# anguswilliams91/bpl-next

Measured on NVIDIA B200. Metric: logdensity_grad_match_evals_per_s, higher is better.
Workload: dtype f32

## Files before the change

bpl_next_b200/csrc/api.cu:

```cuda
#include <limits.h>
#include <stdarg.h>
#include <stdlib.h>
#include <string.h>

#include <algorithm>
#include <atomic>
#include <mutex>
#include <new>

#include "common.cuh"
#include "plan.h"
#include "problem.h"
#include "loo.h"
#include "score_grid.h"
#include "simulate.h"

namespace bplx {

static thread_local char g_err[1024] = "";
static std::atomic<unsigned long long> g_launches{0};

void set_error(const char* fmt, ...) {
  va_list ap;
  va_start(ap, fmt);
  vsnprintf(g_err, sizeof g_err, fmt, ap);
  va_end(ap);
}
void note_launch(int n) { g_launches.fetch_add((unsigned long long)n, std::memory_order_relaxed); }

static EnvSwitches g_env;
static std::once_flag g_env_once;
void reload_env_switches() {
  EnvSwitches e;
  e.no_pdl = getenv("BPLX_NO_PDL") != nullptr;
  e.nuts_generic = getenv("BPLX_NUTS_GENERIC") != nullptr;
  e.no_tail_split = getenv("BPLX_NO_TAIL_SPLIT") != nullptr;
  e.no_transpose = getenv("BPLX_NO_TRANSPOSE") != nullptr;
  if (const char* v = getenv("BPLX_TRANSPOSE_MIN_ELEMS")) e.transpose_min_elems = (size_t)atoll(v);
  if (const char* v = getenv("BPLX_SPLIT")) e.split = atoi(v);
  if (const char* v = getenv("BPLX_HOST_CHUNKS")) e.host_chunks = atoi(v);
  g_env = e;
}
const EnvSwitches& env_switches() {
  std::call_once(g_env_once, reload_env_switches);
  return g_env;
}

constexpr size_t kUploadSlack = (size_t)kMaxSplit * kMaxWarps * sizeof(EntryClip) + 64;
template <typename T>
static int upload(bplx_problem* p, const std::vector<T>& h, const T** out) {
  *out = nullptr;
  if (h.empty()) return BPLX_OK;
  void* d = nullptr;
  const size_t bytes = h.size() * sizeof(T);
  BPLX_CUDA(cudaMalloc(&d, bytes + kUploadSlack));
  p->dev_allocs.push_back(d);
  BPLX_CUDA(cudaMemcpy(d, h.data(), bytes, cudaMemcpyHostToDevice));
  BPLX_CUDA(cudaMemset(static_cast<unsigned char*>(d) + bytes, 0, kUploadSlack));
  *out = static_cast<const T*>(d);
  return BPLX_OK;
}

static float* mapped_or(float* host, float* fallback) {
  cudaPointerAttributes a{};
  if (cudaPointerGetAttributes(&a, host) != cudaSuccess) {
    cudaGetLastError();
    return fallback;
  }
  if (a.type == cudaMemoryTypeHost && a.devicePointer != nullptr) return static_cast<float*>(a.devicePointer);
  return fallback;
}

__global__ void __launch_bounds__(256) transpose_kernel(const float* __restrict__ in, float* __restrict__ out, int R, int Cc,
                                                        size_t ldi, size_t ldo) {
  __shared__ float tile[4][32][33];
  const int c0 = blockIdx.x * 32, r0 = blockIdx.y * 128;
  float v[4][4];
#pragma unroll
  for (int s = 0; s < 4; s++)
#pragma unroll
    for (int k = 0; k < 4; k++) {
      const int r = r0 + s * 32 + threadIdx.y + 8 * k, c = c0 + threadIdx.x;
      v[s][k] = (r < R && c < Cc) ? in[(size_t)r * ldi + c] : 0.0f;
    }
#pragma unroll
  for (int s = 0; s < 4; s++)
#pragma unroll
    for (int k = 0; k < 4; k++) tile[s][threadIdx.y + 8 * k][threadIdx.x] = v[s][k];
  __syncthreads();
#pragma unroll
  for (int s = 0; s < 4; s++)
#pragma unroll
    for (int k = 0; k < 4; k++) {
      const int c = c0 + threadIdx.y + 8 * k, r = r0 + s * 32 + threadIdx.x;
      if (r < R && c < Cc) out[(size_t)c * ldo + r] = tile[s][threadIdx.x][threadIdx.y + 8 * k];
    }
}
static int launch_transpose(const float* in, float* out, int R, int Cc, size_t ldi, size_t ldo, cudaStream_t s) {
  const dim3 grid((unsigned)((Cc + 31) / 32), (unsigned)((R + 127) / 128));
  BPLX_REQUIRE(grid.y <= 65535u, BPLX_E_UNSUPPORTED, "transpose of %d rows", R);
  transpose_kernel<<<grid, dim3(32, 8), 0, s>>>(in, out, R, Cc, ldi, ldo);
  BPLX_CUDA(cudaGetLastError());
  note_launch(1);
  return BPLX_OK;
}

static size_t align256(size_t n) { return (n + 255) / 256 * 256; }
static size_t transpose_room(const KernelParams& kp, int C) {
  if ((size_t)C * (size_t)kp.D < env_switches().transpose_min_elems) return 0;
  return 2 * (((size_t)C + 31) / 32 * 32) * (size_t)kp.D * sizeof(float);
}

static size_t workspace_bytes(const KernelParams& kp, int C) {
  const size_t Cpad = ((size_t)C + 31) / 32 * 32;
  if (kp.model == BPLX_DYNAMIC)
    return ((size_t)kp.G * kp.T * 2 + (kp.dyn_hyp_ws ? (size_t)kp.G * 16 : 0)) * Cpad * sizeof(float);
  if (kp.Cf <= 0) return 0;
  return (size_t)kp.V * Cpad * sizeof(float);
}

static int enqueue(const bplx_problem* p, int C, int layout, int ld, const float* theta, float* lp, float* grad,
                   float* corr_coef, void* ws, size_t ws_bytes, cudaStream_t stream, bool pdl = false, bool lik = false) {
  BPLX_REQUIRE(p != nullptr, BPLX_E_INVALID, "problem is NULL");
  BPLX_REQUIRE(C > 0, BPLX_E_INVALID, "num_chains must be positive (got %d)", C);
  BPLX_REQUIRE(theta && lp && grad, BPLX_E_INVALID, "theta, lp and grad must not be NULL");
  if (layout == BPLX_CHAIN_MAJOR && !env_switches().no_transpose) {
    const size_t base = align256(workspace_bytes(p->kp, C)), room = transpose_room(p->kp, C);
    if (room > 0 && ws != nullptr && ws_bytes >= base + room) {
      const int Dc = lik ? p->lik_D : p->kp.D;
      const size_t ldm = ld > 0 ? (size_t)ld : (size_t)Dc, Cpad = ((size_t)C + 31) / 32 * 32;
      BPLX_REQUIRE(ldm >= (size_t)Dc, BPLX_E_INVALID, "chain-major ld (%d) < D (%d)", ld, Dc);
      float* tin = reinterpret_cast<float*>(static_cast<char*>(ws) + base);
      float* tout = tin + Cpad * (size_t)p->kp.D;
      int rc = launch_transpose(theta, tin, C, Dc, ldm, Cpad, stream);
      if (rc != BPLX_OK) return rc;
      rc = enqueue(p, C, BPLX_CHAIN_MINOR, (int)Cpad, tin, lp, tout, corr_coef, ws, base, stream, pdl, lik);
      if (rc != BPLX_OK) return rc;
      return launch_transpose(tout, grad, Dc, C, Cpad, ldm, stream);
    }
  }
  KernelParams kp = p->kp;
  if (lik) {
    BPLX_REQUIRE(kp.model != BPLX_DYNAMIC, BPLX_E_UNSUPPORTED, "bplx_loglik_fwdbwd: DYNAMIC is not supported");
    kp.lik_only = 1;
    kp.off = p->lik_off;
    for (int i = 0; i < 12; i++) kp.hyper[i] = p->lik_hyper[i];
    kp.nhyper = p->lik_nhyper;
    kp.D = p->lik_D;
    kp.K = 0;
    kp.const_term = p->lik_const;
  }
  if (layout == BPLX_CHAIN_MAJOR) {
    kp.sd = 1;
    kp.sc = ld > 0 ? ld : kp.D;
    BPLX_REQUIRE(kp.sc >= kp.D, BPLX_E_INVALID, "chain-major ld (%d) < D (%d)", ld, kp.D);
  } else if (layout == BPLX_CHAIN_MINOR) {
    kp.sc = 1;
    kp.sd = ld > 0 ? ld : C;
    BPLX_REQUIRE(kp.sd >= C, BPLX_E_INVALID, "chain-minor ld (%d) < num_chains (%d)", ld, C);
  } else {
    BPLX_REQUIRE(false, BPLX_E_INVALID, "unknown layout %d", layout);
  }
  BPLX_REQUIRE((long long)kp.D * (long long)kp.sd + (long long)C * (long long)kp.sc < (1ll << 31), BPLX_E_UNSUPPORTED,
               "theta / grad of %d x %d elements exceed the 31-bit element index of the kernel", C, kp.D);
  const size_t need = workspace_bytes(kp, C);
  BPLX_REQUIRE(ws_bytes >= need && (need == 0 || ws != nullptr), BPLX_E_WORKSPACE,
               "workspace too small: %zu bytes given, %zu needed", ws_bytes, need);
  kp.C = C;
  kp.Cpad = (C + 31) / 32 * 32;
  kp.theta = theta;
  kp.lp = lp;
  kp.grad = grad;
  kp.corr_coef = corr_coef;
  kp.scratch = static_cast<float*>(ws);
  int si = 0;
  const int groups = (C + kChains - 1) / kChains;
  for (int i = kNumSplits - 1; i >= 1; i--)
    if (p->s1[i] && (1 << i) <= kp.split_hint && groups <= p->max_clusters[i]) {
      si = i;
      break;
    }
  if (const int want = env_switches().split) {
    for (int i = 0; i < kNumSplits; i++)
      if ((1 << i) == want && p->s1[i] && (i == 0 || p->max_clusters[i] > 0)) si = i;
  }
  auto use_split = [&](int i) {
    kp.split = 1 << i;
    kp.stream1 = p->s1[i];
    kp.stream2 = p->s2[i];
    kp.warp_b1 = p->wb1[i];
    kp.warp_b2 = p->wb2[i];
  };
  use_split(si);
  kp.group0 = 0;
  kp.ngroups = groups;
  if (kp.model == BPLX_DYNAMIC) return launch_logdensity_dynamic(kp, stream);
  int ti = 0;
  const int rest = p->sm_count > 0 ? groups % p->sm_count : 0;
  if (si == 0 && rest > 0 && rest < groups && !env_switches().split && !env_switches().no_tail_split) {
    for (int i = kNumSplits - 1; i >= 1; i--)
      if (p->s1[i] && (1 << i) <= kp.split_hint && rest <= p->max_clusters[i] && rest * (1 << i) <= p->sm_count) {
        ti = i;
        break;
      }
  }
  if (ti == 0) return launch_logdensity(kp, p->wb[si], stream, pdl);
  kp.ngroups = groups - rest;
  int rc = launch_logdensity(kp, p->wb[0], stream, pdl);
  if (rc != BPLX_OK) return rc;
  use_split(ti);
  kp.group0 = groups - rest;
  kp.ngroups = rest;
  return launch_logdensity(kp, p->wb[ti], stream, pdl);
}

}

using namespace bplx;

extern "C" {

int bplx_problem_create(const bplx_problem_desc* desc, bplx_problem** out) {
  BPLX_REQUIRE(desc && out, BPLX_E_INVALID, "desc / out is NULL");
  *out = nullptr;
  HostPlan hp;
  std::string err;
  int rc = build_plan(*desc, &hp, &err);
  if (rc != BPLX_OK) {
    set_error("%s", err.c_str());
    return rc;
  }
  bplx_problem* p = new (std::nothrow) bplx_problem();
  BPLX_REQUIRE(p, BPLX_E_NOMEM, "out of host memory");
  auto fail = [&](int code) {
    bplx_problem_destroy(p);
    return code;
  };
  if (cudaGetDevice(&p->device) != cudaSuccess) {
    set_error("cudaGetDevice failed: no usable CUDA device (bplx has no CPU fallback)");
    return fail(BPLX_E_CUDA);
  }
  p->kp = hp.kp;
  p->layout = hp.layout;
  p->lik_off = hp.lik_off;
  for (int i = 0; i < 12; i++) p->lik_hyper[i] = hp.lik_hyper[i];
  p->lik_nhyper = hp.lik_nhyper;
  p->lik_D = hp.lik_D;
  p->lik_const = hp.lik_const;
  p->lik_layout = hp.lik_layout;
  KernelParams& kp = p->kp;
#define UP(vec, ptr)                                 \
  if ((rc = upload(p, hp.vec, &(ptr))) != BPLX_OK) return fail(rc)
  UP(stream1, p->s1[0]);
  UP(stream2, p->s2[0]);
  UP(warp_b1, p->wb1[0]);
  UP(warp_b2, p->wb2[0]);
  for (int i = 1; i < kNumSplits; i++) {
    if (hp.more[i - 1].stream1.empty()) continue;
    UP(more[i - 1].stream1, p->s1[i]);
    UP(more[i - 1].stream2, p->s2[i]);
    UP(more[i - 1].warp_b1, p->wb1[i]);
    UP(more[i - 1].warp_b2, p->wb2[i]);
  }
  auto keep_bounds = [&](int i, const std::vector<uint32_t>& b1, const std::vector<uint32_t>& b2) {
    const size_t cap = sizeof(p->wb[i].b1) / sizeof(uint32_t);
    for (size_t k = 0; k < b1.size() && k < cap; k++) p->wb[i].b1[k] = b1[k];
    for (size_t k = 0; k < b2.size() && k < cap; k++) p->wb[i].b2[k] = b2[k];
  };
  keep_bounds(0, hp.warp_b1, hp.warp_b2);
  for (int i = 1; i < kNumSplits; i++) keep_bounds(i, hp.more[i - 1].warp_b1, hp.more[i - 1].warp_b2);
  kp.stream1 = p->s1[0];
  kp.stream2 = p->s2[0];
  kp.warp_b1 = p->wb1[0];
  kp.warp_b2 = p->wb2[0];
  kp.split = 1;
  UP(team_vptr, kp.team_vptr);
  UP(team_flags, kp.team_flags);
  UP(v_team, kp.v_team);
  UP(v_conf, kp.v_conf);
  UP(conf_vptr, kp.conf_vptr);
  UP(conf_vlist, kp.conf_vlist);
  UP(yexp, kp.yexp);
  UP(yteam, kp.yteam);
  UP(yconf, kp.yconf);
  UP(Xs, kp.Xs);
  UP(gw_tptr, kp.gw_tptr);
  UP(gw_tlist, kp.gw_tlist);
#undef UP
  rc = kp.model == BPLX_DYNAMIC ? logdensity_dynamic_set_attributes() : logdensity_set_attributes(kp);
  if (rc != BPLX_OK) return fail(rc);
  if (cudaDeviceGetAttribute(&p->sm_count, cudaDevAttrMultiProcessorCount, p->device) != cudaSuccess) p->sm_count = 0;
  p->max_clusters[0] = 1 << 30;
  if (kp.model != BPLX_DYNAMIC)
    for (int i = 1; i < kNumSplits; i++) p->max_clusters[i] = p->s1[i] ? logdensity_max_clusters(kp, 1 << i) : 0;
  p->stats[0] = desc->num_matches;
  p->stats[1] = hp.n1;
  p->stats[2] = hp.n1_padded;
  p->stats[3] = hp.n2;
  p->stats[4] = hp.n2_padded;
  p->stats[5] = kp.smem_total;
  p->stats[6] = kp.nwarps;
  p->stats[7] = kp.V;
  if (kp.model != BPLX_DYNAMIC) {
    p->warp_stats.assign((size_t)kp.nwarps * 12, 0);
    for (int phase = 0; phase < 2; phase++) {
      const std::vector<unsigned char>& S = phase ? hp.stream2 : hp.stream1;
      const std::vector<uint32_t>& wb = phase ? hp.warp_b2 : hp.warp_b1;
      const size_t esz = (phase == 0 && kp.clip) ? sizeof(EntryClip) : sizeof(Entry);
      const uint32_t minp = phase ? kp.min_piece2 : kp.min_piece1;
      for (int w = 0; w < kp.nwarps && w + 1 < (int)wb.size(); w++) {
        long long* o = &p->warp_stats[(size_t)w * 12 + phase * 6];
        const uint32_t len = wb[w + 1] - wb[w];
        o[5] = (len + kp.stage_bytes - 1) / kp.stage_bytes;
        for (uint32_t st = 0; st < len; st += kp.stage_bytes) {
          uint32_t a = wb[w] + st;
          const uint32_t aend = wb[w] + std::min(len, st + kp.stage_bytes);
          while (a + minp <= aend) {
            ListHdr H;
            memcpy(&H, &S[a], sizeof H);
            if (H.n0 + H.n1 + H.n2 == 0) break;
            const bool home = (H.kind & 1) == 0;
            if (phase == 0) {
              o[home ? 0 : 1]++;
              o[home ? 2 : 3] += H.n0;
            } else {
              o[0]++;
              o[1] += H.n0;
              o[2] += H.n1;
              o[3] += H.n2;
            }
            if (H.flags & kTeamFirst) o[4]++;
            a += (uint32_t)sizeof(ListHdr) + (uint32_t)((H.n0 + H.n1 + H.n2) * esz);
          }
        }
      }
    }
  }
  *out = p;
  return BPLX_OK;
}

void bplx_problem_destroy(bplx_problem* p) {
  if (!p) return;
  for (void* d : p->dev_allocs) cudaFree(d);
  if (p->d_theta) cudaFree(p->d_theta);
  if (p->d_out) cudaFree(p->d_out);
  if (p->d_ws) cudaFree(p->d_ws);
  if (p->d_tin) cudaFree(p->d_tin);
  if (p->d_tout) cudaFree(p->d_tout);
  if (p->host_stream) cudaStreamDestroy(p->host_stream);
  if (p->host_in) cudaStreamDestroy(p->host_in);
  if (p->host_out) cudaStreamDestroy(p->host_out);
  for (cudaEvent_t e : p->host_ev)
    if (e) cudaEventDestroy(e);
  delete p;
}

int bplx_num_params(const bplx_problem* p) { return p ? p->kp.D : BPLX_E_INVALID; }

const char* bplx_problem_layout(const bplx_problem* p) { return p ? p->layout.c_str() : ""; }

int bplx_problem_stats(const bplx_problem* p, long long* out, int n) {
  BPLX_REQUIRE(p && out, BPLX_E_INVALID, "problem / out is NULL");
  for (int i = 0; i < n && i < 8; i++) out[i] = p->stats[i];
  return n < 8 ? n : 8;
}

int bplx_problem_warp_stats(const bplx_problem* p, long long* out, int n) {
  BPLX_REQUIRE(p && out, BPLX_E_INVALID, "problem / out is NULL");
  const int have = (int)p->warp_stats.size();
  for (int i = 0; i < n && i < have; i++) out[i] = p->warp_stats[i];
  return n < have ? n : have;
}

size_t bplx_logdensity_workspace_bytes(const bplx_problem* p, int num_chains) {
  if (!p || num_chains <= 0) return 0;
  const size_t room = transpose_room(p->kp, num_chains);
  return room ? align256(workspace_bytes(p->kp, num_chains)) + room : workspace_bytes(p->kp, num_chains);
}

int bplx_logdensity_fwdbwd(const bplx_problem* p, int num_chains, int layout, int ld, const float* theta, float* lp,
                           float* grad, float* corr_coef, void* workspace, size_t workspace_bytes, void* stream) {
  return enqueue(p, num_chains, layout, ld, theta, lp, grad, corr_coef, workspace, workspace_bytes,
                 static_cast<cudaStream_t>(stream), true);
}

int bplx_loglik_num_inputs(const bplx_problem* p) {
  if (!p) return BPLX_E_INVALID;
  return p->kp.model == BPLX_DYNAMIC ? BPLX_E_UNSUPPORTED : p->lik_D;
}

const char* bplx_loglik_layout(const bplx_problem* p) { return p ? p->lik_layout.c_str() : ""; }

int bplx_loglik_fwdbwd(const bplx_problem* p, int num_chains, int layout, int ld, const float* tables, float* loglik,
                       float* grad, float* corr_coef, void* workspace, size_t workspace_bytes, void* stream) {
  return enqueue(p, num_chains, layout, ld, tables, loglik, grad, corr_coef, workspace, workspace_bytes,
                 static_cast<cudaStream_t>(stream), true, true);
}

int bplx_logdensity_fwdbwd_host(bplx_problem* p, int C, const float* theta, float* lp, float* grad, float* corr_coef) {
  BPLX_REQUIRE(p != nullptr, BPLX_E_INVALID, "problem is NULL");
  BPLX_REQUIRE(C > 0, BPLX_E_INVALID, "num_chains must be positive (got %d)", C);
  BPLX_REQUIRE(theta && lp && grad, BPLX_E_INVALID, "theta, lp and grad must not be NULL");
  std::lock_guard<std::mutex> lock(p->mu);
  BPLX_CUDA(cudaSetDevice(p->device));
  const size_t D = (size_t)p->kp.D;
  if (!p->host_stream) BPLX_CUDA(cudaStreamCreateWithFlags(&p->host_stream, cudaStreamNonBlocking));
  if (C > p->host_cap) {
    if (p->d_theta) cudaFree(p->d_theta);
    if (p->d_out) cudaFree(p->d_out);
    if (p->d_ws) cudaFree(p->d_ws);
    p->d_theta = p->d_out = nullptr;
    p->d_ws = nullptr;
    p->host_cap = 0;
    BPLX_CUDA(cudaMalloc(&p->d_theta, (size_t)C * D * sizeof(float)));
    BPLX_CUDA(cudaMalloc(&p->d_out, ((size_t)C * D + 2 * (size_t)C) * sizeof(float)));
    p->d_ws_bytes = workspace_bytes(p->kp, C);
    if (p->d_ws_bytes) BPLX_CUDA(cudaMalloc(&p->d_ws, p->d_ws_bytes));
    p->host_cap = C;
  }
  if (!p->host_in) {
    BPLX_CUDA(cudaStreamCreateWithFlags(&p->host_in, cudaStreamNonBlocking));
    BPLX_CUDA(cudaStreamCreateWithFlags(&p->host_out, cudaStreamNonBlocking));
    for (cudaEvent_t& e : p->host_ev) BPLX_CUDA(cudaEventCreateWithFlags(&e, cudaEventDisableTiming));
  }
  cudaStream_t s = p->host_stream;
  float* d_grad = p->d_out;
  float* d_lp = p->d_out + (size_t)C * D;
  float* d_cc = d_lp + C;
  const size_t payload = (size_t)C * D * sizeof(float);
  int nchunk = payload >= ((size_t)80 << 20) ? 8 : (payload >= ((size_t)16 << 20) ? 4 : (payload >= ((size_t)6 << 20) ? 2 : 1));
  while (nchunk > 1 && C / nchunk < 256) nchunk /= 2;
  if (const int want = env_switches().host_chunks)
    if (want == 1 || want == 2 || want == 4 || want == 8 || want == 16) nchunk = want;
  const bool native = (size_t)C * D >= std::max(env_switches().transpose_min_elems, (size_t)1 << 20) && !env_switches().no_transpose;
  if (nchunk == 1) {
    float* k_lp = mapped_or(lp, d_lp);
    float* k_cc = corr_coef ? mapped_or(corr_coef, d_cc) : d_cc;
    BPLX_CUDA(cudaMemcpyAsync(p->d_theta, theta, (size_t)C * D * sizeof(float), cudaMemcpyHostToDevice, s));
    int rc;
    if (native) {
      const int ldc = (C + 31) / 32 * 32;
      if (ldc > p->tr_cap) {
        if (p->d_tin) cudaFree(p->d_tin);
        if (p->d_tout) cudaFree(p->d_tout);
        p->d_tin = p->d_tout = nullptr;
        p->tr_cap = 0;
        BPLX_CUDA(cudaMalloc(&p->d_tin, (size_t)ldc * D * sizeof(float)));
        BPLX_CUDA(cudaMalloc(&p->d_tout, (size_t)ldc * D * sizeof(float)));
        p->tr_cap = ldc;
      }
      rc = launch_transpose(p->d_theta, p->d_tin, C, (int)D, D, (size_t)ldc, s);
      if (rc != BPLX_OK) return rc;
      rc = enqueue(p, C, BPLX_CHAIN_MINOR, ldc, p->d_tin, k_lp, p->d_tout, k_cc, p->d_ws, p->d_ws_bytes, s);
      if (rc != BPLX_OK) return rc;
      rc = launch_transpose(p->d_tout, d_grad, (int)D, C, (size_t)ldc, D, s);
    } else {
      rc = enqueue(p, C, BPLX_CHAIN_MAJOR, (int)D, p->d_theta, k_lp, d_grad, k_cc, p->d_ws, p->d_ws_bytes, s);
    }
    if (rc != BPLX_OK) return rc;
    BPLX_CUDA(cudaMemcpyAsync(grad, d_grad, (size_t)C * D * sizeof(float), cudaMemcpyDeviceToHost, s));
    if (k_lp == d_lp) BPLX_CUDA(cudaMemcpyAsync(lp, d_lp, (size_t)C * sizeof(float), cudaMemcpyDeviceToHost, s));
    if (corr_coef && k_cc == d_cc)
      BPLX_CUDA(cudaMemcpyAsync(corr_coef, d_cc, (size_t)C * sizeof(float), cudaMemcpyDeviceToHost, s));
    BPLX_CUDA(cudaStreamSynchronize(s));
    return BPLX_OK;
  }
  const int per = ((C + nchunk - 1) / nchunk + 31) / 32 * 32;
  if (native && per > p->tr_cap) {
    if (p->d_tin) cudaFree(p->d_tin);
    if (p->d_tout) cudaFree(p->d_tout);
    p->d_tin = p->d_tout = nullptr;
    p->tr_cap = 0;
    BPLX_CUDA(cudaMalloc(&p->d_tin, (size_t)per * D * sizeof(float)));
    BPLX_CUDA(cudaMalloc(&p->d_tout, (size_t)per * D * sizeof(float)));
    p->tr_cap = per;
  }
  int sizes[40], ns = 0, left = C;
  auto push = [&](int n) {
    n = n < left ? n : left;
    if (n > 0) sizes[ns++] = n, left -= n;
  };
  if (nchunk >= 4) {
    const int half = (per / 2 + 31) / 32 * 32;
    push(half);
    push(half);
    while (left > per) push(per);
    push((left / 2 + 31) / 32 * 32);
    push(left);
  } else {
    while (left > 0) push(per);
  }
  for (int k = 0, c0 = 0; k < ns; c0 += sizes[k], k++) {
    const int n = sizes[k];
    const size_t off = (size_t)c0 * D;
    BPLX_CUDA(cudaMemcpyAsync(p->d_theta + off, theta + off, (size_t)n * D * sizeof(float), cudaMemcpyHostToDevice, p->host_in));
    BPLX_CUDA(cudaEventRecord(p->host_ev[2 * k], p->host_in));
    BPLX_CUDA(cudaStreamWaitEvent(s, p->host_ev[2 * k], 0));
    int rc;
    if (native) {
      rc = launch_transpose(p->d_theta + off, p->d_tin, n, (int)D, D, (size_t)per, s);
      if (rc != BPLX_OK) return rc;
      rc = enqueue(p, n, BPLX_CHAIN_MINOR, per, p->d_tin, d_lp + c0, p->d_tout, d_cc + c0, p->d_ws, p->d_ws_bytes, s);
      if (rc != BPLX_OK) return rc;
      rc = launch_transpose(p->d_tout, d_grad + off, (int)D, n, (size_t)per, D, s);
    } else {
      rc = enqueue(p, n, BPLX_CHAIN_MAJOR, (int)D, p->d_theta + off, d_lp + c0, d_grad + off, d_cc + c0, p->d_ws,
                   p->d_ws_bytes, s);
    }
    if (rc != BPLX_OK) return rc;
    BPLX_CUDA(cudaEventRecord(p->host_ev[2 * k + 1], s));
    BPLX_CUDA(cudaStreamWaitEvent(p->host_out, p->host_ev[2 * k + 1], 0));
    BPLX_CUDA(cudaMemcpyAsync(grad + off, d_grad + off, (size_t)n * D * sizeof(float), cudaMemcpyDeviceToHost, p->host_out));
    BPLX_CUDA(cudaMemcpyAsync(lp + c0, d_lp + c0, (size_t)n * sizeof(float), cudaMemcpyDeviceToHost, p->host_out));
    if (corr_coef)
      BPLX_CUDA(cudaMemcpyAsync(corr_coef + c0, d_cc + c0, (size_t)n * sizeof(float), cudaMemcpyDeviceToHost, p->host_out));
  }
  BPLX_CUDA(cudaStreamSynchronize(p->host_out));
  return BPLX_OK;
}

static int check_sample_args(const bplx_samples* s, const bplx_fixtures* f, const char* what,
                             bool allow_no_fixtures = false) {
  BPLX_REQUIRE(s && f, BPLX_E_INVALID, "samples / fixtures is NULL");
  BPLX_REQUIRE(s->model >= BPLX_DIXON_COLES && s->model <= BPLX_NEUTRAL_WC, BPLX_E_UNSUPPORTED,
               "%s: model %d unsupported (DYNAMIC predict is unusable in the reference)", what, s->model);
  const bool fixtures = !(allow_no_fixtures && f->num_fixtures == 0);
  BPLX_REQUIRE(s->num_samples > 0 && s->num_teams > 0 && (f->num_fixtures > 0 || !fixtures), BPLX_E_INVALID,
               "%s: num_samples, num_teams and num_fixtures must be positive", what);
  BPLX_REQUIRE(s->attack && s->defence && s->corr_coef && (!fixtures || (f->home_team && f->away_team)), BPLX_E_INVALID,
               "%s: attack, defence, corr_coef, home_team, away_team must not be NULL", what);
  BPLX_REQUIRE(s->home_attack, BPLX_E_INVALID, "%s: home_attack (home advantage) must not be NULL", what);
  if (s->model == BPLX_NEUTRAL || s->model == BPLX_NEUTRAL_WC)
    BPLX_REQUIRE(s->away_attack && s->home_defence && s->away_defence, BPLX_E_INVALID,
                 "%s: neutral models need away_attack, home_defence, away_defence", what);
  if (s->model == BPLX_NEUTRAL_WC)
    BPLX_REQUIRE(s->confederation_strength && s->num_conferences > 0 && (!fixtures || (f->home_conf && f->away_conf)),
                 BPLX_E_INVALID, "%s: NEUTRAL_WC needs confederation_strength, home_conf, away_conf", what);
  return BPLX_OK;
}

static int check_grid_args(const bplx_samples* s, const bplx_fixtures* f, int max_goals) {
  const int rc = check_sample_args(s, f, "score grid");
  if (rc != BPLX_OK) return rc;
  BPLX_REQUIRE(max_goals >= 1 && max_goals <= 63, BPLX_E_INVALID, "max_goals must be in [1, 63] (got %d)", max_goals);
  return BPLX_OK;
}

static size_t grid_plan(const bplx_samples* s, const bplx_fixtures* f, int max_goals, GridParams* gp, const char** err) {
  gp->model = s->model;
  gp->S = s->num_samples;
  gp->T = s->num_teams;
  gp->Cf = s->model == BPLX_NEUTRAL_WC ? s->num_conferences : 0;
  gp->F = f->num_fixtures;
  gp->g = max_goals + 1;
  return score_grid_plan(gp, err);
}

size_t bplx_score_grid_workspace_bytes(const bplx_samples* s, const bplx_fixtures* f, int max_goals) {
  if (!s || !f || max_goals < 1 || s->num_samples <= 0 || s->num_teams <= 0 || f->num_fixtures <= 0) return 0;
  GridParams gp{};
  return grid_plan(s, f, max_goals, &gp, nullptr);
}

int bplx_score_grid(const bplx_samples* s, const bplx_fixtures* f, int max_goals, float scale, float* grid,
                    float* outcome, void* workspace, size_t workspace_bytes, void* stream) {
  return bplx_score_grid_ex(s, f, max_goals, scale, grid, outcome, workspace, workspace_bytes, stream, 0u);
}

int bplx_score_grid_ex(const bplx_samples* s, const bplx_fixtures* f, int max_goals, float scale, float* grid,
                       float* outcome, void* workspace, size_t workspace_bytes, void* stream, unsigned flags) {
  int rc = check_grid_args(s, f, max_goals);
  if (rc != BPLX_OK) return rc;
  BPLX_REQUIRE(grid != nullptr, BPLX_E_INVALID, "grid is NULL");
  GridParams gp{};
  const char* perr = nullptr;
  const size_t need = grid_plan(s, f, max_goals, &gp, &perr);
  BPLX_REQUIRE(need > 0, BPLX_E_UNSUPPORTED, "%s", perr ? perr : "score grid: unsupported shape");
  gp.scale = scale;
  BPLX_REQUIRE(workspace && workspace_bytes >= need, BPLX_E_WORKSPACE,
               "workspace too small: %zu bytes given, %zu needed", workspace_bytes, need);
  BPLX_REQUIRE((reinterpret_cast<uintptr_t>(workspace) & 15u) == 0, BPLX_E_INVALID, "workspace must be 16-byte aligned");
  gp.attack = s->attack;
  gp.defence = s->defence;
  gp.ha = s->home_attack;
  gp.aa = s->away_attack;
  gp.hd = s->home_defence;
  gp.ad = s->away_defence;
  gp.conf = s->confederation_strength;
  gp.corr = s->corr_coef;
  gp.home = f->home_team;
  gp.away = f->away_team;
  gp.hconf = f->home_conf;
  gp.aconf = f->away_conf;
  gp.nv = f->neutral_venue;
  gp.table = static_cast<float*>(workspace);
  gp.partial = reinterpret_cast<float*>(static_cast<unsigned char*>(workspace) +
                                        ((size_t)gp.S * gp.row_floats * 4 + 255) / 256 * 256);
  gp.grid = grid;
  gp.outcome = outcome;
  gp.reuse_tables = (flags & BPLX_GRID_REUSE_TABLES) ? 1 : 0;
  return launch_score_grid(gp, static_cast<cudaStream_t>(stream));
}

int bplx_score_grid_host(const bplx_samples* s, const bplx_fixtures* f, int max_goals, float scale, float* grid,
                         float* outcome) {
  int rc = check_grid_args(s, f, max_goals);
  if (rc != BPLX_OK) return rc;
  BPLX_REQUIRE(grid != nullptr, BPLX_E_INVALID, "grid is NULL");
  const size_t S = s->num_samples, T = s->num_teams, F = f->num_fixtures, g = max_goals + 1;
  const size_t Cf = s->model == BPLX_NEUTRAL_WC ? s->num_conferences : 0;
  for (size_t i = 0; i < F; i++) {
    BPLX_REQUIRE(f->home_team[i] < T && f->away_team[i] < T, BPLX_E_INVALID,
                 "score grid: team index out of range at fixture %zu (%u, %u; num_teams %zu)", i,
                 (unsigned)f->home_team[i], (unsigned)f->away_team[i], T);
    if (Cf)
      BPLX_REQUIRE(f->home_conf[i] < Cf && f->away_conf[i] < Cf, BPLX_E_INVALID,
                   "score grid: confederation index out of range at fixture %zu (%u, %u; num_conferences %zu)", i,
                   (unsigned)f->home_conf[i], (unsigned)f->away_conf[i], Cf);
  }
  std::vector<void*> allocs;
  auto cleanup = [&]() {
    for (void* d : allocs) cudaFree(d);
  };
  cudaStream_t st = nullptr;
  if (cudaStreamCreateWithFlags(&st, cudaStreamNonBlocking) != cudaSuccess) {
    set_error("cudaStreamCreate failed: no usable CUDA device (bplx has no CPU fallback)");
    return BPLX_E_CUDA;
  }
  rc = BPLX_OK;
  auto up = [&](const void* h, size_t bytes) -> void* {
    if (!h || rc != BPLX_OK) return nullptr;
    void* d = nullptr;
    if (cudaMalloc(&d, bytes) != cudaSuccess ||
        cudaMemcpyAsync(d, h, bytes, cudaMemcpyHostToDevice, st) != cudaSuccess) {
      set_error("score_grid_host: device allocation / copy of %zu bytes failed", bytes);
      rc = BPLX_E_CUDA;
      return nullptr;
    }
    allocs.push_back(d);
    return d;
  };
  bplx_samples ds = *s;
  bplx_fixtures df = *f;
  const size_t ha_w = s->model == BPLX_DIXON_COLES ? 1 : T;
  ds.attack = (const float*)up(s->attack, S * T * 4);
  ds.defence = (const float*)up(s->defence, S * T * 4);
  ds.home_attack = (const float*)up(s->home_attack, S * ha_w * 4);
  const bool neu = s->model == BPLX_NEUTRAL || s->model == BPLX_NEUTRAL_WC;
  ds.away_attack = neu ? (const float*)up(s->away_attack, S * T * 4) : nullptr;
  ds.home_defence = neu ? (const float*)up(s->home_defence, S * T * 4) : nullptr;
  ds.away_defence = neu ? (const float*)up(s->away_defence, S * T * 4) : nullptr;
  ds.confederation_strength = Cf ? (const float*)up(s->confederation_strength, S * Cf * 4) : nullptr;
  ds.corr_coef = (const float*)up(s->corr_coef, S * 4);
  df.home_team = (const uint16_t*)up(f->home_team, F * 2);
  df.away_team = (const uint16_t*)up(f->away_team, F * 2);
  df.home_conf = Cf ? (const uint8_t*)up(f->home_conf, F) : nullptr;
  df.away_conf = Cf ? (const uint8_t*)up(f->away_conf, F) : nullptr;
  df.neutral_venue = (neu && f->neutral_venue) ? (const uint8_t*)up(f->neutral_venue, F) : nullptr;
  const size_t ws_bytes = bplx_score_grid_workspace_bytes(s, f, max_goals);
  void *d_ws = nullptr, *d_grid = nullptr, *d_out = nullptr;
  if (rc == BPLX_OK) {
    if (cudaMalloc(&d_ws, ws_bytes) == cudaSuccess) allocs.push_back(d_ws); else rc = BPLX_E_NOMEM;
    if (cudaMalloc(&d_grid, F * g * g * 4) == cudaSuccess) allocs.push_back(d_grid); else rc = BPLX_E_NOMEM;
    if (outcome) {
      if (cudaMalloc(&d_out, F * 3 * 4) == cudaSuccess) allocs.push_back(d_out); else rc = BPLX_E_NOMEM;
    }
    if (rc != BPLX_OK) set_error("score_grid_host: out of device memory");
  }
  if (rc == BPLX_OK)
    rc = bplx_score_grid(&ds, &df, max_goals, scale, (float*)d_grid, (float*)d_out, d_ws, ws_bytes, st);
  if (rc == BPLX_OK) {
    cudaError_t e = cudaMemcpyAsync(grid, d_grid, F * g * g * 4, cudaMemcpyDeviceToHost, st);
    if (e == cudaSuccess && outcome) e = cudaMemcpyAsync(outcome, d_out, F * 3 * 4, cudaMemcpyDeviceToHost, st);
    if (e == cudaSuccess) e = cudaStreamSynchronize(st);
    if (e != cudaSuccess) {
      set_error("score_grid_host: %s", cudaGetErrorString(e));
      rc = BPLX_E_CUDA;
    }
  } else {
    cudaStreamSynchronize(st);
  }
  cleanup();
  cudaStreamDestroy(st);
  return rc;
}

static size_t pointwise_plan_for(const bplx_samples* s, const bplx_observations* o, PointwiseParams* pp, const char** err) {
  pp->gp.model = s->model;
  pp->gp.S = s->num_samples;
  pp->gp.T = s->num_teams;
  pp->gp.Cf = s->model == BPLX_NEUTRAL_WC ? s->num_conferences : 0;
  pp->gp.F = o->fixtures.num_fixtures;
  return pointwise_plan(pp, err);
}

size_t bplx_pointwise_loglik_workspace_bytes(const bplx_samples* s, const bplx_observations* obs) {
  if (!s || !obs || s->num_samples <= 0 || s->num_teams <= 0 || obs->fixtures.num_fixtures <= 0) return 0;
  PointwiseParams pp{};
  return pointwise_plan_for(s, obs, &pp, nullptr);
}

int bplx_pointwise_loglik(const bplx_samples* s, const bplx_observations* obs, float* loglik, size_t ld, double* stats,
                          void* workspace, size_t workspace_bytes, void* stream) {
  BPLX_REQUIRE(obs != nullptr, BPLX_E_INVALID, "observations is NULL");
  int rc = check_sample_args(s, &obs->fixtures, "pointwise log-likelihood");
  if (rc != BPLX_OK) return rc;
  BPLX_REQUIRE(obs->home_goals && obs->away_goals, BPLX_E_INVALID,
               "pointwise log-likelihood: home_goals and away_goals must not be NULL");
  BPLX_REQUIRE(stats != nullptr, BPLX_E_INVALID, "pointwise log-likelihood: stats is NULL");
  BPLX_REQUIRE(!loglik || ld >= (size_t)s->num_samples, BPLX_E_INVALID,
               "pointwise log-likelihood: ld (%zu) < num_samples (%d)", ld, s->num_samples);
  PointwiseParams pp{};
  const char* perr = nullptr;
  const size_t need = pointwise_plan_for(s, obs, &pp, &perr);
  BPLX_REQUIRE(need > 0, BPLX_E_UNSUPPORTED, "%s", perr ? perr : "pointwise log-likelihood: unsupported shape");
  BPLX_REQUIRE(workspace && workspace_bytes >= need, BPLX_E_WORKSPACE,
               "workspace too small: %zu bytes given, %zu needed", workspace_bytes, need);
  BPLX_REQUIRE((reinterpret_cast<uintptr_t>(workspace) & 15u) == 0, BPLX_E_INVALID, "workspace must be 16-byte aligned");
  GridParams& gp = pp.gp;
  gp.attack = s->attack;
  gp.defence = s->defence;
  gp.ha = s->home_attack;
  gp.aa = s->away_attack;
  gp.hd = s->home_defence;
  gp.ad = s->away_defence;
  gp.conf = s->confederation_strength;
  gp.corr = s->corr_coef;
  gp.home = obs->fixtures.home_team;
  gp.away = obs->fixtures.away_team;
  gp.hconf = obs->fixtures.home_conf;
  gp.aconf = obs->fixtures.away_conf;
  gp.nv = obs->fixtures.neutral_venue;
  gp.table = static_cast<float*>(workspace);
  pp.partial = reinterpret_cast<double*>(static_cast<unsigned char*>(workspace) +
                                         ((size_t)gp.S * gp.row_floats * 4 + 255) / 256 * 256);
  pp.hg = obs->home_goals;
  pp.ag = obs->away_goals;
  pp.ll = loglik;
  pp.ld = ld;
  pp.stats = stats;
  return launch_pointwise(pp, static_cast<cudaStream_t>(stream));
}

int bplx_psis_loo(const float* loglik, int num_matches, int num_samples, size_t ld, double r_eff, double* elpd_i,
                  double* pareto_k, void* workspace, size_t workspace_bytes, void* stream) {
  (void)workspace;
  (void)workspace_bytes;
  BPLX_REQUIRE(loglik && elpd_i && pareto_k, BPLX_E_INVALID, "psis loo: loglik, elpd_i and pareto_k must not be NULL");
  BPLX_REQUIRE(num_matches > 0 && num_samples > 0, BPLX_E_INVALID,
               "psis loo: num_matches and num_samples must be positive (got %d, %d)", num_matches, num_samples);
  BPLX_REQUIRE(ld >= (size_t)num_samples, BPLX_E_INVALID, "psis loo: ld (%zu) < num_samples (%d)", ld, num_samples);
  BPLX_REQUIRE(r_eff > 0.0 && r_eff <= 1e300, BPLX_E_INVALID, "psis loo: r_eff must be positive and finite (got %g)", r_eff);
  PsisParams pp{};
  pp.Mt = psis_tail_length(num_samples, r_eff);
  BPLX_REQUIRE(pp.Mt <= kPsisTailMax, BPLX_E_UNSUPPORTED,
               "psis loo: a tail of %d draws (ceil(min(0.2 S, 3 sqrt(S / r_eff)))) exceeds the kernel's limit of %d "
               "(BPLX_PSIS_MAX_TAIL)", pp.Mt, kPsisTailMax);
  pp.cap = 8;
  while (pp.cap < pp.Mt) pp.cap <<= 1;
  pp.ll = loglik;
  pp.ld = ld;
  pp.M = num_matches;
  pp.S = num_samples;
  pp.elpd = elpd_i;
  pp.khat = pareto_k;
  return launch_psis(pp, static_cast<cudaStream_t>(stream));
}

static size_t simulate_plan_for(const bplx_samples* s, const bplx_fixtures* f, SimParams* sp) {
  sp->gp.model = s->model;
  sp->gp.S = s->num_samples;
  sp->gp.T = s->num_teams;
  sp->gp.Cf = s->model == BPLX_NEUTRAL_WC ? s->num_conferences : 0;
  sp->gp.F = f->num_fixtures;
  return simulate_plan(sp);
}

size_t bplx_simulate_workspace_bytes(const bplx_samples* s, const bplx_fixtures* f, const bplx_table* t) {
  if (!s || !f || !t || s->num_samples <= 0 || s->num_teams <= 0 || f->num_fixtures <= 0) return 0;
  SimParams sp{};
  return simulate_plan_for(s, f, &sp);
}

static int simulate_setup(const bplx_samples* s, const bplx_fixtures* f, const uint8_t* home_slot,
                          const uint8_t* away_slot, const bplx_table* t, int max_goals, int sims_per_draw,
                          unsigned long long seed, long long first_draw, unsigned long long* position_counts,
                          unsigned long long* points_counts, uint8_t* positions, uint8_t* scores,
                          unsigned long long* invalid, const char* what, bool allow_no_fixtures, SimParams* out) {
  int rc = check_sample_args(s, f, what, allow_no_fixtures);
  if (rc != BPLX_OK) return rc;
  BPLX_REQUIRE(t != nullptr, BPLX_E_INVALID, "%s: table is NULL", what);
  BPLX_REQUIRE(t->num_slots <= BPLX_SIM_MAX_TEAMS, BPLX_E_UNSUPPORTED,
               "%s: %d table slots exceed the kernel's limit of %d (BPLX_SIM_MAX_TEAMS)", what, t->num_slots,
               BPLX_SIM_MAX_TEAMS);
  BPLX_REQUIRE(t->num_slots >= 1, BPLX_E_INVALID, "%s: the table needs at least one slot", what);
  BPLX_REQUIRE(t->num_positions >= 1 && t->num_positions <= t->num_slots && t->num_points_bins >= 1, BPLX_E_INVALID,
               "%s: num_positions must be in [1, num_slots] and num_points_bins >= 1 (got %d, %d)", what,
               t->num_positions, t->num_points_bins);
  BPLX_REQUIRE(t->points_win >= 1 && t->points_draw >= 0 && t->points_draw <= t->points_win, BPLX_E_INVALID,
               "%s: points must satisfy 0 <= points_draw <= points_win, points_win >= 1 (got %d, %d)", what,
               t->points_win, t->points_draw);
  BPLX_REQUIRE(t->start_points && t->start_goals_for && t->start_goals_against, BPLX_E_INVALID,
               "%s: start_points, start_goals_for and start_goals_against must not be NULL", what);
  BPLX_REQUIRE((home_slot && away_slot) || f->num_fixtures == 0, BPLX_E_INVALID,
               "%s: home_slot and away_slot must not be NULL", what);
  BPLX_REQUIRE(max_goals >= 1 && max_goals <= 63, BPLX_E_INVALID, "%s: max_goals must be in [1, 63] (got %d)", what,
               max_goals);
  BPLX_REQUIRE(sims_per_draw >= 1, BPLX_E_INVALID, "%s: sims_per_draw must be >= 1 (got %d)", what, sims_per_draw);
  BPLX_REQUIRE(first_draw >= 0 && first_draw + s->num_samples <= LLONG_MAX / sims_per_draw, BPLX_E_INVALID,
               "%s: first_draw must be >= 0 and (first_draw + num_samples) * sims_per_draw must fit 63 bits", what);
  BPLX_REQUIRE((long long)s->num_samples * sims_per_draw <= INT_MAX, BPLX_E_UNSUPPORTED,
               "%s: num_samples * sims_per_draw must be below 2^31 per call (got %lld): cut the draws into ranges",
               what, (long long)s->num_samples * sims_per_draw);
  BPLX_REQUIRE(position_counts && points_counts && invalid, BPLX_E_INVALID,
               "%s: position_counts, points_counts and invalid must not be NULL", what);
  SimParams& sp = *out;
  GridParams& gp = sp.gp;
  gp.attack = s->attack;
  gp.defence = s->defence;
  gp.ha = s->home_attack;
  gp.aa = s->away_attack;
  gp.hd = s->home_defence;
  gp.ad = s->away_defence;
  gp.conf = s->confederation_strength;
  gp.corr = s->corr_coef;
  gp.home = f->home_team;
  gp.away = f->away_team;
  gp.hconf = f->home_conf;
  gp.aconf = f->away_conf;
  gp.nv = f->neutral_venue;
  sp.hslot = home_slot;
  sp.aslot = away_slot;
  sp.group = t->group;
  sp.start_pts = t->start_points;
  sp.start_gf = t->start_goals_for;
  sp.start_ga = t->start_goals_against;
  sp.NT = t->num_slots;
  sp.P = t->num_positions;
  sp.B = t->num_points_bins;
  sp.G = max_goals;
  sp.R = sims_per_draw;
  sp.pw = t->points_win;
  sp.pd = t->points_draw;
  sp.seed = seed;
  sp.first_draw = first_draw;
  sp.N = s->num_samples * sims_per_draw;
  sp.pos_counts = position_counts;
  sp.pts_counts = points_counts;
  sp.invalid = invalid;
  sp.positions = positions;
  sp.scores = scores;
  return BPLX_OK;
}

int bplx_simulate_table(const bplx_samples* s, const bplx_fixtures* f, const uint8_t* home_slot, const uint8_t* away_slot,
                        const bplx_table* t, int max_goals, int sims_per_draw, unsigned long long seed,
                        long long first_draw, unsigned long long* position_counts, unsigned long long* points_counts,
                        uint8_t* positions, uint8_t* scores, unsigned long long* invalid, void* workspace,
                        size_t workspace_bytes, void* stream) {
  SimParams sp{};
  int rc = simulate_setup(s, f, home_slot, away_slot, t, max_goals, sims_per_draw, seed, first_draw, position_counts,
                          points_counts, positions, scores, invalid, "simulate", false, &sp);
  if (rc != BPLX_OK) return rc;
  const size_t need = simulate_plan_for(s, f, &sp);
  BPLX_REQUIRE(workspace && workspace_bytes >= need, BPLX_E_WORKSPACE,
               "workspace too small: %zu bytes given, %zu needed", workspace_bytes, need);
  BPLX_REQUIRE((reinterpret_cast<uintptr_t>(workspace) & 15u) == 0, BPLX_E_INVALID, "workspace must be 16-byte aligned");
  sp.gp.table = static_cast<float*>(workspace);
  return launch_simulate(sp, static_cast<cudaStream_t>(stream));
}

static size_t alloc_bytes(const bplx_bracket* b) {
  return b->best_alloc ? ((size_t)b->best_count << b->num_groups) : 0;
}

size_t bplx_simulate_tournament_workspace_bytes(const bplx_samples* s, const bplx_fixtures* f, const bplx_table* t,
                                                const bplx_bracket* b) {
  if (!s || !f || !t || !b || s->num_samples <= 0 || s->num_teams <= 0 || f->num_fixtures < 0) return 0;
  if (b->num_groups < 0 || b->num_groups > BPLX_SIM_MAX_TEAMS || b->best_count < 0) return 0;
  if (b->best_alloc && b->num_groups > BPLX_KO_MAX_ALLOC_GROUPS) return 0;
  SimParams sp{};
  return simulate_plan_for(s, f, &sp) + (alloc_bytes(b) + 255) / 256 * 256;
}

static int check_bracket(const bplx_bracket* b, const bplx_samples* s, int NT, int P, KoParams* ko) {
  BPLX_REQUIRE(b != nullptr, BPLX_E_INVALID, "tournament: bracket is NULL");
  const int K = b->num_ties;
  BPLX_REQUIRE(K >= 1, BPLX_E_INVALID, "tournament: the bracket needs at least one tie (got %d)", K);
  BPLX_REQUIRE(K <= BPLX_KO_MAX_TIES, BPLX_E_UNSUPPORTED,
               "tournament: %d ties exceed the kernel's limit of %d (BPLX_KO_MAX_TIES)", K, BPLX_KO_MAX_TIES);
  BPLX_REQUIRE(b->num_rounds >= 1 && b->num_rounds <= BPLX_KO_MAX_ROUNDS, BPLX_E_UNSUPPORTED,
               "tournament: num_rounds must be in [1, %d] (got %d)", BPLX_KO_MAX_ROUNDS, b->num_rounds);
  BPLX_REQUIRE(b->num_groups >= 0 && b->num_groups <= NT, BPLX_E_INVALID,
               "tournament: num_groups must be in [0, num_slots] (got %d)", b->num_groups);
  BPLX_REQUIRE(b->best_count >= 0 && b->best_count <= BPLX_KO_MAX_BEST, BPLX_E_UNSUPPORTED,
               "tournament: best_count must be in [0, %d] (got %d)", BPLX_KO_MAX_BEST, b->best_count);
  BPLX_REQUIRE(b->best_count <= b->num_groups, BPLX_E_INVALID,
               "tournament: best_count (%d) exceeds num_groups (%d)", b->best_count, b->num_groups);
  BPLX_REQUIRE(b->best_count == 0 || (b->best_position >= 0 && b->best_position < P), BPLX_E_INVALID,
               "tournament: best_position must be in [0, num_positions) (got %d)", b->best_position);
  BPLX_REQUIRE(b->kind && b->arg0 && b->arg1 && b->round && b->slot_team, BPLX_E_INVALID,
               "tournament: kind, arg0, arg1, round and slot_team must not be NULL");
  BPLX_REQUIRE(s->model != BPLX_NEUTRAL_WC || b->slot_conf, BPLX_E_INVALID, "tournament: NEUTRAL_WC needs slot_conf");
  for (int t = 0; t < NT; t++) {
    BPLX_REQUIRE(b->slot_team[t] < s->num_teams, BPLX_E_INVALID,
                 "tournament: slot_team[%d] = %d is not a model team (T = %d)", t, b->slot_team[t], s->num_teams);
    if (s->model == BPLX_NEUTRAL_WC)
      BPLX_REQUIRE(b->slot_conf[t] < s->num_conferences, BPLX_E_INVALID,
                   "tournament: slot_conf[%d] = %d is not a confederation (Cf = %d)", t, b->slot_conf[t],
                   s->num_conferences);
  }
  for (int k = 0; k < K; k++) {
    BPLX_REQUIRE(b->round[k] < b->num_rounds, BPLX_E_INVALID, "tournament: tie %d: round %d >= num_rounds (%d)", k,
                 b->round[k], b->num_rounds);
    for (int side = 0; side < 2; side++) {
      const int kind = b->kind[2 * k + side], a0 = b->arg0[2 * k + side], a1 = b->arg1[2 * k + side];
      const char* sd = side ? "away" : "home";
      switch (kind) {
        case BPLX_ENTRANT_SLOT:
          BPLX_REQUIRE(a0 < NT, BPLX_E_INVALID, "tournament: tie %d %s: slot %d outside the table (%d slots)", k, sd,
                       a0, NT);
          break;
        case BPLX_ENTRANT_GROUP_POS:
          BPLX_REQUIRE(a0 < b->num_groups && a1 < P, BPLX_E_INVALID,
                       "tournament: tie %d %s: group %d position %d out of range (%d groups, %d positions)", k, sd, a0,
                       a1, b->num_groups, P);
          break;
        case BPLX_ENTRANT_BEST:
          BPLX_REQUIRE(a0 < b->best_count, BPLX_E_INVALID, "tournament: tie %d %s: BEST %d >= best_count (%d)", k, sd,
                       a0, b->best_count);
          break;
        case BPLX_ENTRANT_WINNER:
        case BPLX_ENTRANT_LOSER:
          BPLX_REQUIRE(a0 < k, BPLX_E_INVALID, "tournament: tie %d %s: refers to tie %d, which is not earlier", k, sd,
                       a0);
          break;
        default:
          BPLX_REQUIRE(false, BPLX_E_INVALID, "tournament: tie %d %s: unknown entrant kind %d", k, sd, kind);
      }
      ko->kind[side][k] = (uint8_t)kind;
      ko->arg0[side][k] = (uint8_t)a0;
      ko->arg1[side][k] = (uint8_t)a1;
    }
    ko->round[k] = b->round[k];
    ko->neutral[k] = b->neutral_venue ? (b->neutral_venue[k] != 0) : 0;
  }
  if (b->best_alloc) {
    BPLX_REQUIRE(b->best_count >= 1, BPLX_E_INVALID, "tournament: an allocation table needs best_count >= 1");
    BPLX_REQUIRE(b->num_groups <= BPLX_KO_MAX_ALLOC_GROUPS, BPLX_E_UNSUPPORTED,
                 "tournament: an allocation table supports at most %d groups (got %d)", BPLX_KO_MAX_ALLOC_GROUPS,
                 b->num_groups);
    for (unsigned mask = 0; mask < (1u << b->num_groups); mask++) {
      unsigned seen = 0;
      for (int j = 0; j < b->best_count; j++) {
        const int g = b->best_alloc[(size_t)mask * b->best_count + j];
        if (g == 0xFF) continue;
        BPLX_REQUIRE(g < b->num_groups && ((mask >> g) & 1u) && !((seen >> g) & 1u), BPLX_E_INVALID,
                     "tournament: allocation row 0x%x entry %d: group %d is not a distinct group of the row's set", mask,
                     j, g);
        seen |= 1u << g;
      }
    }
  }
  for (int t = 0; t < NT; t++) {
    ko->slot_team[t] = b->slot_team[t];
    ko->slot_conf[t] = b->slot_conf ? b->slot_conf[t] : 0;
  }
  ko->K = K;
  ko->nr = b->num_rounds;
  ko->ng = b->num_groups;
  ko->bp = b->best_position;
  ko->bc = b->best_count;
  return BPLX_OK;
}

int bplx_simulate_tournament(const bplx_samples* s, const bplx_fixtures* f, const uint8_t* home_slot,
                             const uint8_t* away_slot, const bplx_table* t, const bplx_bracket* b, int max_goals,
                             int sims_per_draw, unsigned long long seed, long long first_draw,
                             unsigned long long* position_counts, unsigned long long* points_counts,
                             unsigned long long* reach_counts, unsigned long long* win_counts, uint8_t* positions,
                             uint8_t* scores, uint8_t* ko_entrants, uint8_t* ko_scores, uint8_t* ko_winners,
                             unsigned long long* invalid, void* workspace, size_t workspace_bytes, void* stream) {
  SimParams sp{};
  int rc = simulate_setup(s, f, home_slot, away_slot, t, max_goals, sims_per_draw, seed, first_draw, position_counts,
                          points_counts, positions, scores, invalid, "tournament", true, &sp);
  if (rc != BPLX_OK) return rc;
  rc = check_bracket(b, s, t->num_slots, t->num_positions, &sp.ko);
  if (rc != BPLX_OK) return rc;
  BPLX_REQUIRE(reach_counts && win_counts, BPLX_E_INVALID, "tournament: reach_counts and win_counts must not be NULL");
  const size_t table = simulate_plan_for(s, f, &sp);
  const size_t need = table + (alloc_bytes(b) + 255) / 256 * 256;
  BPLX_REQUIRE(workspace && workspace_bytes >= need, BPLX_E_WORKSPACE,
               "workspace too small: %zu bytes given, %zu needed", workspace_bytes, need);
  BPLX_REQUIRE((reinterpret_cast<uintptr_t>(workspace) & 15u) == 0, BPLX_E_INVALID, "workspace must be 16-byte aligned");
  sp.gp.table = static_cast<float*>(workspace);
  sp.ko.reach = reach_counts;
  sp.ko.win = win_counts;
  sp.ko.entrants = ko_entrants;
  sp.ko.scores = ko_scores;
  sp.ko.winners = ko_winners;
  if (b->best_alloc) {
    uint8_t* const dst = static_cast<uint8_t*>(workspace) + table;
    BPLX_CUDA(cudaMemcpyAsync(dst, b->best_alloc, alloc_bytes(b), cudaMemcpyHostToDevice,
                              static_cast<cudaStream_t>(stream)));
    sp.ko.alloc = dst;
  }
  return launch_simulate_tournament(sp, static_cast<cudaStream_t>(stream));
}

void bplx_reload_env(void) {
  env_switches();
  reload_env_switches();
}
const char* bplx_last_error(void) { return g_err; }
int bplx_version(void) { return BPLX_VERSION; }
unsigned long long bplx_launch_count(void) { return g_launches.load(std::memory_order_relaxed); }

}
```

bpl_next_b200/csrc/k1_common.cuh:

```cuda
#pragma once
#include <float.h>

#include "common.cuh"
#include "plan.h"

namespace bplx {

namespace {


constexpr float kLn2 = 0.693147180559945309f;
constexpr unsigned kFull = 0xffffffffu;

struct Hyp {
  float mu_d, sig_a, sig_d, mu[4], sig[4];
};

struct Lane {
  const float* th;
  float* gr;
  float* sc;
  int sd;
  bool active;
  __device__ __forceinline__ float ld(int d) const { return __ldg(th + (uint32_t)(d * sd)); }
  __device__ __forceinline__ float* g(int d) const { return gr + (uint32_t)(d * sd); }
};

__device__ __forceinline__ float sigmoid_clipped(float x) {
  float s = 1.0f / (1.0f + expf(-x));
  return fminf(fmaxf(s, FLT_MIN), 1.0f - FLT_EPSILON);
}
__device__ __forceinline__ float rcp_approx(float x) {
  float y;
  asm("rcp.approx.ftz.f32 %0, %1;" : "=f"(y) : "f"(x));
  return y;
}
__device__ __forceinline__ float lg2_approx(float x) {
  float y;
  asm("lg2.approx.ftz.f32 %0, %1;" : "=f"(y) : "f"(x));
  return y;
}
__device__ __forceinline__ void red_add(float* p, float v) {
  asm volatile("red.global.add.f32 [%0], %1;" ::"l"(p), "f"(v) : "memory");
}
__device__ __forceinline__ float ld_cg(const float* p) { return __ldcg(p); }

__device__ __forceinline__ Hyp load_hyp_raw(const KernelParams& kp, const Lane& ln) {
  const ThetaOffsets& o = kp.off;
  Hyp hy;
  if (kp.lik_only) {
    hy.mu_d = hy.sig_a = hy.sig_d = 0.0f;
#pragma unroll
    for (int i = 0; i < 4; i++) {
      hy.mu[i] = o.mean[i] >= 0 ? ln.ld(o.mean[i]) : 0.0f;
      hy.sig[i] = 0.0f;
    }
    return hy;
  }
  hy.mu_d = ln.ld(o.mean_defence);
  hy.sig_a = ln.ld(o.log_std_attack);
  hy.sig_d = ln.ld(o.log_std_defence);
#pragma unroll
  for (int i = 0; i < 4; i++) {
    hy.mu[i] = o.mean[i] >= 0 ? ln.ld(o.mean[i]) : 0.0f;
    hy.sig[i] = o.log_std[i] >= 0 ? ln.ld(o.log_std[i]) : 0.0f;
  }
  return hy;
}
__device__ __forceinline__ Hyp finish_hyp(const KernelParams& kp, Hyp hy) {
  const ThetaOffsets& o = kp.off;
  hy.sig_a = expf(hy.sig_a);
  hy.sig_d = expf(hy.sig_d);
#pragma unroll
  for (int i = 0; i < 4; i++) hy.sig[i] = (o.log_std[i] >= 0 || (kp.lik_only && i < kp.ndec)) ? expf(hy.sig[i]) : 0.0f;
  return hy;
}
__device__ __forceinline__ Hyp load_hyp(const KernelParams& kp, const Lane& ln) { return finish_hyp(kp, load_hyp_raw(kp, ln)); }

struct Hdr {
  uint32_t own_off, vteam, kind, flags, n0, n1, n2, team;
};
__device__ __forceinline__ Hdr unpack_hdr(const uint4 h) {
  Hdr H;
  H.own_off = h.x;
  H.vteam = h.y & 0xffffu;
  H.kind = (h.y >> 16) & 0xffu;
  H.flags = h.y >> 24;
  H.n0 = h.z & 0xffffu;
  H.n1 = h.z >> 16;
  H.n2 = h.w & 0xffffu;
  H.team = h.w >> 16;
  return H;
}

__device__ __forceinline__ void add_own(float (&g)[6], uint32_t kind, float gx, float gy) {
  if (kind == kH1) {
    g[eAh1] += gx; g[eBh1] += gy;
  } else if (kind == kA1) {
    g[eBa1] += gx; g[eAa1] += gy;
  } else {
    g[eB0] += gx; g[eA0] += gy;
  }
}

template <bool ADD>
__device__ __forceinline__ void put_raw(const KernelParams& kp, const Lane& ln, int t, const float (&g)[6], float& hacc) {
  const ThetaOffsets& o = kp.off;
  const float ra = g[eAh1] + g[eAa1] + g[eA0];
  const float rd = -(g[eBh1] + g[eBa1] + g[eB0]);
  const float rx[4] = {g[eAh1], g[eAa1], -g[eBh1], -g[eBa1]};
  if (kp.ndec == 0) hacc += rx[0];
  if (!ln.active) return;
  if (ADD) {
    red_add(ln.g(o.za + t), ra);
    red_add(ln.g(o.zd + t), rd);
  } else {
    *ln.g(o.za + t) = ra;
    *ln.g(o.zd + t) = rd;
  }
#pragma unroll
  for (int i = 0; i < 4; i++) {
    if (i < kp.ndec) {
      if (ADD) red_add(ln.g(o.dec[i] + t), rx[i]);
      else *ln.g(o.dec[i] + t) = rx[i];
    }
  }
}

__device__ __forceinline__ void put_side(const KernelParams& kp, float* q, const float (&g)[6], float& hacc) {
  q[0] = g[eAh1] + g[eAa1] + g[eA0];
  q[32] = -(g[eBh1] + g[eBa1] + g[eB0]);
  const float rx[4] = {g[eAh1], g[eAa1], -g[eBh1], -g[eBa1]};
  if (kp.ndec == 0) hacc += rx[0];
#pragma unroll
  for (int i = 0; i < 4; i++)
    if (i < kp.ndec) q[(2 + i) * 32] = rx[i];
}

struct Ring {
  uint32_t ring, bar;
  uint32_t S;
  const unsigned char* src;
  uint32_t total;
  uint32_t gs0, gs_next;
  int lane;

  __device__ __forceinline__ void init(uint32_t ring_, uint32_t bar_, uint32_t S_, int lane_) {
    ring = ring_; bar = bar_; S = S_; lane = lane_;
    total = gs0 = gs_next = 0;
    src = nullptr;
    if (lane == 0) {
#pragma unroll
      for (int s = 0; s < kStages; s++) mbar_init(bar + 8 * s, 1);
      fence_mbar_init();
      fence_proxy_async();
    }
    __syncwarp();
  }
  __device__ __forceinline__ void issue(uint32_t k) {
    const uint32_t b0 = k * S;
    if (lane == 0 && b0 < total) {
      const uint32_t bytes = min(S, total - b0);
      const uint32_t slot = (gs0 + k) % kStages;
      mbar_arrive_expect_tx(bar + 8 * slot, bytes);
      tma_load_1d(ring + slot * S, src + b0, bytes, bar + 8 * slot);
    }
  }
  __device__ __forceinline__ void begin(const void* src_, uint32_t total_bytes) {
    __syncwarp();
    src = static_cast<const unsigned char*>(src_);
    total = total_bytes;
    gs0 = gs_next;
    gs_next = gs0 + (total_bytes + S - 1) / S;
#pragma unroll
    for (int s = 0; s < kStages; s++) issue(s);
  }
  __device__ __forceinline__ uint32_t num_stages() const { return (total + S - 1) / S; }
  __device__ __forceinline__ uint32_t acquire(uint32_t k, uint32_t* bytes) {
    const uint32_t idx = gs0 + k, slot = idx % kStages;
    mbar_wait(bar + 8 * slot, (idx / kStages) & 1);
    *bytes = min(S, total - k * S);
    return ring + slot * S;
  }
  __device__ __forceinline__ void release(uint32_t k) {
    __syncwarp();
    issue(k + kStages);
  }
};

template <typename F>
__device__ __forceinline__ void walk16(uint32_t& a, const uint32_t e_end, F&& item) {
  while (a + 64 <= e_end) {
    item(a);
    item(a + 16);
    item(a + 32);
    item(a + 48);
    a += 64;
  }
  if (a + 32 <= e_end) {
    item(a);
    item(a + 16);
    a += 32;
  }
  if (a < e_end) {
    item(a);
    a += 16;
  }
}

enum { kTauPlain = 0, kTauUnclipped = 1, kTauClipped = 2 };
template <int MODE>
__device__ __forceinline__ void tau_piece(uint32_t& a, const Hdr& L, const float2 own, const bool home, const float cc,
                                          const uint32_t tab, float& lt_out, float& du_out, float& gx_out, float& gy_out) {
  const float2 one = make_float2(1.0f, 1.0f);
  float2 lt = make_float2(0.0f, 0.0f), uxy = lt, sxy_x = lt, sxy_y = lt;
  {
    const uint32_t e_end = a + L.n0 * (uint32_t)sizeof(Entry);
#pragma unroll 2
    for (; a < e_end; a += 16) {
      const uint4 q = lds128u(a);
      const float2 ea = lds64(tab + q.x), eb = lds64(tab + q.z);
      const float2 w = make_float2(__uint_as_float(q.y), __uint_as_float(q.w));
      const float2 ra = mul2(own, ea), rb = mul2(own, eb);
      float2 t;
      if (MODE == kTauClipped) t = make_float2(fminf(ra.x, 15.0f) * fminf(ra.y, 15.0f), fminf(rb.x, 15.0f) * fminf(rb.y, 15.0f));
      else t = make_float2(ra.x * ra.y, rb.x * rb.y);
      float2 tau = fma2(bc2(-cc), t, one);
      tau.x = fmaxf(tau.x, 0.0f);
      tau.y = fmaxf(tau.y, 0.0f);
      const float2 wt = mul2(w, t), rc = make_float2(rcp_approx(tau.x), rcp_approx(tau.y));
      uxy = fma2(wt, rc, uxy);
      if (MODE == kTauClipped) {
        if (ra.x < 15.0f) sxy_x.x = fmaf(wt.x, rc.x, sxy_x.x);
        if (rb.x < 15.0f) sxy_x.y = fmaf(wt.y, rc.y, sxy_x.y);
        if (ra.y < 15.0f) sxy_y.x = fmaf(wt.x, rc.x, sxy_y.x);
        if (rb.y < 15.0f) sxy_y.y = fmaf(wt.y, rc.y, sxy_y.y);
      }
      if (home) lt = fma2(w, make_float2(lg2_approx(tau.x), lg2_approx(tau.y)), lt);
    }
  }
  float u1[2] = {0.0f, 0.0f}, s1[2] = {0.0f, 0.0f};
#pragma unroll
  for (int c = 0; c < 2; c++) {
    const float oc = c == 0 ? own.x : own.y;
    const uint32_t e_end = a + (c == 0 ? L.n1 : L.n2) * (uint32_t)sizeof(Entry);
    float2 u = make_float2(0.0f, 0.0f), sm = u;
#pragma unroll 2
    for (; a < e_end; a += 16) {
      const uint4 q = lds128u(a);
      const float2 Rr = mul2(bc2(oc), make_float2(lds32(tab + q.x), lds32(tab + q.z)));
      const float2 w = make_float2(__uint_as_float(q.y), __uint_as_float(q.w));
      const float2 R = MODE == kTauClipped ? make_float2(fminf(Rr.x, 15.0f), fminf(Rr.y, 15.0f)) : Rr;
      float2 tau = fma2(bc2(cc), R, one);
      tau.x = fmaxf(tau.x, 0.0f);
      tau.y = fmaxf(tau.y, 0.0f);
      const float2 wr = mul2(w, R), rc = make_float2(rcp_approx(tau.x), rcp_approx(tau.y));
      u = fma2(wr, rc, u);
      if (MODE == kTauClipped) {
        if (Rr.x < 15.0f) sm.x = fmaf(wr.x, rc.x, sm.x);
        if (Rr.y < 15.0f) sm.y = fmaf(wr.y, rc.y, sm.y);
      }
      if (home) lt = fma2(w, make_float2(lg2_approx(tau.x), lg2_approx(tau.y)), lt);
    }
    u1[c] = u.x + u.y;
    s1[c] = MODE == kTauClipped ? sm.x + sm.y : u1[c];
  }
  const float uxy_s = uxy.x + uxy.y;
  const float sx = MODE == kTauClipped ? sxy_x.x + sxy_x.y : uxy_s, sy = MODE == kTauClipped ? sxy_y.x + sxy_y.y : uxy_s;
  lt_out = lt.x + lt.y;
  du_out = u1[0] + u1[1] - uxy_s;
  gx_out = cc * (s1[0] - sx);
  gy_out = cc * (s1[1] - sy);
}

struct Fixup {
  uint32_t teams[2];
  uint32_t confs;
  uint32_t vts[2];
  float vx[2], vy[2];
  uint32_t h1;
};

__device__ __forceinline__ void fold_fixup(const Fixup& fx, int which, int side, float& ra, float& rd, float (&rx)[4]) {
  const bool h1 = (fx.h1 >> which) & 1u;
  const float vx = fx.vx[which], vy = fx.vy[which];
  if (side == 0) {
    if (h1) { ra += vx; rx[0] += vx; rd -= vy; rx[2] -= vy; }
    else { rd -= vx; ra += vy; }
  } else {
    if (h1) { rd -= vx; rx[3] -= vx; ra += vy; rx[1] += vy; }
    else { ra += vx; rd -= vy; }
  }
}
__device__ __forceinline__ float fixup_conf(const Fixup& fx, int which, int side) {
  const bool h1 = (fx.h1 >> which) & 1u;
  const float d = fx.vx[which] - fx.vy[which];
  return ((side == 0) == h1) ? d : -d;
}

}

}
```

bpl_next_b200/csrc/logdensity.cu:

```cuda
#include <cooperative_groups.h>

#include <math.h>

#include "k1_common.cuh"
#include "problem.h"

namespace cg = cooperative_groups;

#ifdef BPLX_TIMELINE
__device__ unsigned long long g_timeline[32 * 24];
#define BPLX_STAMP(i)                                                                    \
  do {                                                                                   \
    if (blockIdx.x == 0 && (threadIdx.x & 31) == 0) {                                    \
      unsigned long long t_;                                                             \
      asm volatile("mov.u64 %0, %%globaltimer;" : "=l"(t_));                             \
      g_timeline[(threadIdx.x >> 5) * 24 + (i)] = t_;                                    \
    }                                                                                    \
  } while (0)
#define BPLX_STAMP_DEP(i, dep)                                                           \
  do {                                                                                   \
    if (blockIdx.x == 0 && (threadIdx.x & 31) == 0) {                                    \
      unsigned long long t_;                                                             \
      asm volatile("mov.u64 %0, %%globaltimer;" : "=l"(t_) : "f"(dep));                  \
      g_timeline[(threadIdx.x >> 5) * 24 + (i)] = t_;                                    \
    }                                                                                    \
  } while (0)
#else
#define BPLX_STAMP(i)
#define BPLX_STAMP_DEP(i, dep)
#endif

namespace bplx {

template <bool FAST, bool HOME>
__device__ __forceinline__ void rate_piece_clip(uint32_t& a, const uint32_t e_end, const float2 own, const uint32_t tab,
                                                float& lp, float& m1, float& m2, float& m3, float& gx, float& gy) {
  float2 lg = make_float2(0.0f, 0.0f), lw = lg, g = lg;
  walk16(a, e_end, [&](const uint32_t at) {
    const uint4 q = lds128u(at);
    const float2 ea = lds64(tab + q.x);
    const float w = __uint_as_float(q.y);
    const float2 wy = make_float2(__uint_as_float(q.z), __uint_as_float(q.w));
    const float2 XY = mul2(own, ea);
    const float2 d = fma2(bc2(-w), XY, wy);
    if (FAST) {
      g = add2(g, d);
    } else {
      if (XY.x < 15.0f) g.x += d.x;
      if (XY.y < 15.0f) g.y += d.y;
    }
    if (HOME) {
      const float2 c = FAST ? XY : make_float2(fminf(XY.x, 15.0f), fminf(XY.y, 15.0f));
      lg = fma2(wy, make_float2(lg2_approx(c.x), lg2_approx(c.y)), lg);
      lw = fma2(bc2(w), c, lw);
      m1 = fmaxf(m1, c.x);
      m2 = fmaxf(m2, c.y);
      m3 = fmaxf(m3, c.x * c.y);
    }
  });
  gx = g.x;
  gy = g.y;
  if (HOME) lp = fmaf(lg.x + lg.y, kLn2, -(lw.x + lw.y));
}

__device__ __forceinline__ uint32_t float_key(float f) {
  const uint32_t b = __float_as_uint(f);
  return b ^ ((uint32_t)((int32_t)b >> 31) | 0x80000000u);
}
__device__ __forceinline__ float key_float(uint32_t k) {
  return __uint_as_float(k ^ ((k & 0x80000000u) ? 0x80000000u : 0xffffffffu));
}

template <bool CLIP>
__global__ void __launch_bounds__(kMaxWarps * 32, 1) logdensity_kernel(const __grid_constant__ KernelParams kp,
                                                                        const __grid_constant__ WarpBounds wb) {
  extern __shared__ __align__(1024) unsigned char smem[];
  BPLX_STAMP(19);
  const int lane = threadIdx.x & 31, warp = threadIdx.x >> 5, W = kp.nwarps;
  const ThetaOffsets& o = kp.off;
  const int S = kp.split;
  const int crank = S > 1 ? (int)cg::this_cluster().block_rank() : 0;
  const int group = kp.group0 + (int)blockIdx.x / S;
  const int vwarp = crank * W + warp, VW = S * W;
  auto sync_all = [&]() {
    if (S > 1) cg::this_cluster().sync();
    else __syncthreads();
  };
  const int chain_raw = group * kChains + lane;
  const int chain = min(chain_raw, kp.C - 1);
  Lane ln;
  ln.th = kp.theta + (size_t)chain * (size_t)kp.sc;
  ln.gr = kp.grad + (size_t)chain * (size_t)kp.sc;
  ln.sc = kp.scratch + chain;
  ln.sd = kp.sd;
  ln.active = chain_raw < kp.C;
  const uint32_t tab = smem_u32(smem) + lane * 8;
  unsigned long long* red_best = reinterpret_cast<unsigned long long*>(smem + kp.smem_red);
  unsigned long long* red_found = reinterpret_cast<unsigned long long*>(smem + kp.smem_red + 768);
  float* red_hyp = reinterpret_cast<float*>(smem + kp.smem_red + 1280);
  float* red_gc = reinterpret_cast<float*>(smem + kp.smem_red + 1280 + 12 * 128);
  const uint32_t a_best = cluster_map(smem_u32(red_best), 0), a_found = cluster_map(smem_u32(red_found), 0);
  const uint32_t a_cl = cluster_map(smem_u32(smem) + kp.smem_red_cl, 0);
  const uint32_t a_partcl = cluster_map(smem_u32(smem) + kp.epi_cl, 0);
  const uint32_t a_teamrows = cluster_map(smem_u32(smem) + kp.epi_team, 0);
  constexpr uint32_t ESZ = CLIP ? (uint32_t)sizeof(EntryClip) : (uint32_t)sizeof(Entry);
  Ring ring;
  ring.init(smem_u32(smem) + kp.smem_ring + warp * (kStages * kp.stage_bytes),
            smem_u32(smem) + kp.smem_bar + warp * (kStages * 8), kp.stage_bytes, lane);
  const uint32_t b1_0 = wb.b1[vwarp], b1_1 = wb.b1[vwarp + 1];
  ring.begin(kp.stream1 + b1_0, b1_1 - b1_0);
  pdl_wait();
  pdl_launch_dependents();
  ln.th = after_wait(ln.th);
  ln.gr = after_wait(ln.gr);
  ln.sc = after_wait(ln.sc);
  const int ndec = kp.ndec;
  const bool dc = ndec == 0;
  const float raw_in = ln.ld(o.raw);
  const bool lik = kp.lik_only != 0;
  const float u_in = (warp == 0 && !dc && !lik) ? ln.ld(o.u) : 0.0f;
  struct TeamIn { float za, zd, dz[4], xs[4]; int fl, v0, v1; };
  auto load_team = [&](int t) {
    TeamIn in;
    in.za = ln.ld(o.za + t);
    in.zd = ln.ld(o.zd + t);
#pragma unroll
    for (int i = 0; i < 4; i++) in.dz[i] = i < ndec ? ln.ld(o.dec[i] + t) : 0.0f;
#pragma unroll
    for (int j = 0; j < 4; j++) in.xs[j] = j < kp.K ? __ldg(kp.Xs + (size_t)t * kp.K + j) : 0.0f;
    in.fl = __ldg(kp.team_flags + t);
    in.v0 = __ldg(kp.team_vptr + t);
    in.v1 = __ldg(kp.team_vptr + t + 1);
    return in;
  };
  TeamIn nx = load_team(min(warp, kp.T - 1));
  float ba[4], bd[4];
#pragma unroll
  for (int j = 0; j < 4; j++) {
    ba[j] = j < kp.K ? ln.ld(o.beta_a + j) : 0.0f;
    bd[j] = j < kp.K ? ln.ld(o.beta_d + j) : 0.0f;
  }
  const Hyp hy_in = load_hyp_raw(kp, ln);
  {
    const int nthr = W * 32;
    if (kp.sd == 1) {
      const int per = (kp.D + 31) / 32;
      for (int i = threadIdx.x; i < 32 * per; i += nthr) {
        const int c = min(group * kChains + i / per, kp.C - 1);
        asm volatile("prefetch.global.L2 [%0];" ::"l"(kp.theta + (size_t)c * (size_t)kp.sc + (size_t)(i % per) * 32));
      }
    } else {
      for (int d = threadIdx.x; d < kp.D; d += nthr)
        asm volatile("prefetch.global.L2 [%0];" ::"l"(kp.theta + (size_t)d * (size_t)kp.sd + (size_t)group * kChains));
    }
  }

  float lp_acc = 0.0f;
  float hacc = 0.0f;

  const bool p2s = kp.smem_p2 != 0 && S == 1;
  float* p2_tab = reinterpret_cast<float*>(smem + kp.smem_p2);
  uint32_t* red_clip = reinterpret_cast<uint32_t*>(smem + kp.smem_red_cl);
  if (warp == 0) {
    const uint32_t zr = (uint32_t)kp.V * kRowBytes;
    if (kp.has1) {
      sts64(tab + kp.tabP1 + zr, 0.0f, 0.0f);
      sts64(tab + kp.tabQ1 + zr, 0.0f, 0.0f);
    }
    if (kp.has0) sts64(tab + kp.tabP0 + zr, 0.0f, 0.0f);
    if (CLIP) red_clip[lane] = red_clip[32 + lane] = 0u;
    if (crank == 0) {
      uint32_t* rb = reinterpret_cast<uint32_t*>(red_best);
      rb[lane] = rb[32 + lane] = rb[64 + lane] = 0u;
      rb[96 + lane] = rb[128 + lane] = rb[160 + lane] = 0xffffffffu;
      red_found[lane] = red_found[32 + lane] = ~0ull;
    }
  }
  if (CLIP) __syncthreads();

  BPLX_STAMP(0);
  BPLX_STAMP_DEP(12, raw_in);
  {
    const Hyp hy = finish_hyp(kp, hy_in);
    BPLX_STAMP_DEP(13, hy.sig_a + hy.sig_d + hy.sig[0] + hy.sig[1] + hy.sig[2] + hy.sig[3] + nx.za + nx.zd);
    if (warp == 0) {
      red_hyp[0 * 32 + lane] = hy.mu_d; red_hyp[1 * 32 + lane] = hy.sig_a; red_hyp[2 * 32 + lane] = hy.sig_d;
#pragma unroll
      for (int i = 0; i < 4; i++) { red_hyp[(3 + i) * 32 + lane] = hy.mu[i]; red_hyp[(7 + i) * 32 + lane] = hy.sig[i]; }
    }
    float exA = -FLT_MAX, exB = -FLT_MAX;
    for (int t = warp; t < kp.T; t += W) {
      const TeamIn in = nx;
      if (t + W < kp.T) nx = load_team(t + W);
      if (p2s) {
#pragma unroll
        for (int side = 0; side < 2; side++)
#pragma unroll
          for (int i = 0; i < 6; i++)
            if (i < 2 + ndec) p2_tab[((side * kp.T + t) * (2 + ndec) + i) * 32 + lane] = 0.0f;
      }
      float am = 0.0f, dm = hy.mu_d;
#pragma unroll
      for (int j = 0; j < 4; j++) {
        am = fmaf(in.xs[j], ba[j], am);
        dm = fmaf(in.xs[j], bd[j], dm);
      }
      for (int k = 4; k < kp.K; k++) {
        const float x = __ldg(kp.Xs + (size_t)t * kp.K + k);
        am = fmaf(x, ln.ld(o.beta_a + k), am);
        dm = fmaf(x, ln.ld(o.beta_d + k), dm);
      }
      const float att = fmaf(in.za, hy.sig_a, am), def = fmaf(in.zd, hy.sig_d, dm);
      float x[4] = {dc ? hy.mu[0] : 0.0f, 0.0f, 0.0f, 0.0f};
#pragma unroll
      for (int i = 0; i < 4; i++)
        if (i < ndec) x[i] = fmaf(hy.sig[i], in.dz[i], hy.mu[i]);
      if (!(in.fl & 1) && ln.active && crank == 0) {
        *ln.g(o.za + t) = 0.0f;
        *ln.g(o.zd + t) = 0.0f;
#pragma unroll
        for (int i = 0; i < 4; i++)
          if (i < ndec) *ln.g(o.dec[i] + t) = 0.0f;
      }
      for (int v = in.v0; v < in.v1; v++) {
        const float cf = kp.Cf > 0 ? ln.ld(o.conf + __ldg(kp.v_conf + v)) : 0.0f;
        float ex[6];
        ex[eAh1] = att + x[0] + cf;
        ex[eBh1] = -def - x[2] - cf;
        ex[eBa1] = -def - x[3] - cf;
        ex[eAa1] = att + x[1] + cf;
        ex[eA0] = att + cf;
        ex[eB0] = -def - cf;
        const uint32_t r = (uint32_t)v * kRowBytes;
        if (kp.has1) {
          sts64(tab + kp.tabP1 + r, expf(ex[eAh1]), expf(ex[eBh1]));
          sts64(tab + kp.tabQ1 + r, expf(ex[eBa1]), expf(ex[eAa1]));
        }
        if (kp.has0) sts64(tab + kp.tabP0 + r, expf(ex[eA0]), expf(ex[eB0]));
        if (CLIP) {
          exA = fmaxf(exA, fmaxf(ex[eAh1], fmaxf(ex[eAa1], ex[eA0])));
          exB = fmaxf(exB, fmaxf(ex[eBh1], fmaxf(ex[eBa1], ex[eB0])));
        }
        if (!CLIP && crank == 0) {
#pragma unroll
          for (int e = 0; e < 6; e++) lp_acc = fmaf(__ldg(kp.yexp + (size_t)v * 6 + e), ex[e], lp_acc);
        }
      }
    }
    if (warp == 0) red_hyp[11 * 32 + lane] = (dc || lik) ? 0.5f : sigmoid_clipped(u_in);
    if (CLIP && warp < kp.T) {
      atomicMax(red_clip + lane, float_key(exA));
      atomicMax(red_clip + 32 + lane, float_key(exB));
    }
  }
  const float r = lik ? raw_in : sigmoid_clipped(raw_in);
  BPLX_STAMP(1);
  sync_all();

  BPLX_STAMP(2);
  bool fast1 = false;
  if (CLIP) fast1 = __all_sync(kFull, key_float(red_clip[lane]) + key_float(red_clip[32 + lane]) < 2.707f) && !(kp.force_clip_forms & 1);
  float best[3] = {0.0f, 0.0f, 0.0f};
  uint32_t besth[3] = {0u, 0u, 0u};
  {
    float g[6] = {0.0f, 0.0f, 0.0f, 0.0f, 0.0f, 0.0f}, cacc = 0.0f;
    const uint32_t nst = ring.num_stages();
    for (uint32_t k = 0; k < nst; k++) {
      uint32_t bytes;
      const uint32_t a0 = ring.acquire(k, &bytes);
      if (k == 0) BPLX_STAMP(16);
      uint32_t a = a0;
      const uint32_t aend = a0 + bytes;
      while (a + kp.min_piece1 <= aend) {
        const uint32_t hoff = b1_0 + k * ring.S + (a - a0);
        const Hdr L = unpack_hdr(lds128u(a));
        a += 16;
        const uint32_t e_end = a + L.n0 * ESZ;
        if (L.flags & kTeamFirst) {
#pragma unroll
          for (int e = 0; e < 6; e++) g[e] = 0.0f;
        }
        float2 own = lds64(tab + L.own_off);
        if (L.kind >= kH0) { const float s = own.x; own.x = own.y; own.y = s; }
        const bool home = (L.kind & 1) == 0;
        float gx, gy;
        if (!CLIP) {
          float2 acc0 = make_float2(0.0f, 0.0f), acc1 = acc0;
          if (home) {
            float m1 = 0.0f, m2 = 0.0f, m3 = 0.0f;
            walk16(a, e_end, [&](const uint32_t at) {
              const uint4 q = lds128u(at);
              const float2 ea = lds64(tab + q.x), eb = lds64(tab + q.z);
              acc0 = fma2(bc2(__uint_as_float(q.y)), ea, acc0);
              acc1 = fma2(bc2(__uint_as_float(q.w)), eb, acc1);
              m1 = fmaxf(m1, fmaxf(ea.x, eb.x));
              m2 = fmaxf(m2, fmaxf(ea.y, eb.y));
              m3 = fmaxf(m3, fmaxf(ea.x * ea.y, eb.x * eb.y));
            });
            const float v0 = own.x * m1, v1 = own.y * m2, v2 = (own.x * own.y) * m3;
            if (v0 > best[0]) { best[0] = v0; besth[0] = hoff; }
            if (v1 > best[1]) { best[1] = v1; besth[1] = hoff; }
            if (v2 > best[2]) { best[2] = v2; besth[2] = hoff; }
          } else {
            walk16(a, e_end, [&](const uint32_t at) {
              const uint4 q = lds128u(at);
              const float2 ea = lds64(tab + q.x), eb = lds64(tab + q.z);
              acc0 = fma2(bc2(__uint_as_float(q.y)), ea, acc0);
              acc1 = fma2(bc2(__uint_as_float(q.w)), eb, acc1);
            });
          }
          const float SX = own.x * (acc0.x + acc1.x), SY = own.y * (acc0.y + acc1.y);
          lp_acc -= 0.5f * (SX + SY);
          gx = -SX;
          gy = -SY;
        } else {
          float lp = 0.0f, m1 = 0.0f, m2 = 0.0f, m3 = 0.0f;
          if (fast1) {
            if (home) rate_piece_clip<true, true>(a, e_end, own, tab, lp, m1, m2, m3, gx, gy);
            else rate_piece_clip<true, false>(a, e_end, own, tab, lp, m1, m2, m3, gx, gy);
          } else {
            if (home) rate_piece_clip<false, true>(a, e_end, own, tab, lp, m1, m2, m3, gx, gy);
            else rate_piece_clip<false, false>(a, e_end, own, tab, lp, m1, m2, m3, gx, gy);
          }
          if (home) {
            lp_acc += lp;
            if (m1 > best[0]) { best[0] = m1; besth[0] = hoff; }
            if (m2 > best[1]) { best[1] = m2; besth[1] = hoff; }
            if (m3 > best[2]) { best[2] = m3; besth[2] = hoff; }
          }
        }
        add_own(g, L.kind, gx, gy);
        if (kp.Cf > 0) {
          cacc += L.kind == kH1 ? gx - gy : gy - gx;
          if (L.flags & kVteamLast) {
            if (ln.active) ln.sc[(size_t)L.vteam * kp.Cpad] = cacc;
            cacc = 0.0f;
          }
        }
        if (L.flags & kTeamLast) put_raw<false>(kp, ln, (int)L.team, g, hacc);
        if (k == 0 && a - a0 <= kp.stage_bytes / 2) BPLX_STAMP(17);
      }
      ring.release(k);
    }
  }
  const uint32_t b2_0 = wb.b2[vwarp], b2_1 = wb.b2[vwarp + 1];
  ring.begin(kp.stream2 + b2_0, b2_1 - b2_0);

  BPLX_STAMP(3);
#pragma unroll
  for (int q = 0; q < 3; q++)
    if (best[q] > 0.0f) dsm_atom_max_u32(a_best + (uint32_t)(q * 32 + lane) * 4u, __float_as_uint(best[q]));
  sync_all();
  BPLX_STAMP(14);
#pragma unroll
  for (int q = 0; q < 3; q++) {
    const float gq = __uint_as_float(dsm_ld_u32(a_best + (uint32_t)(q * 32 + lane) * 4u));
    if (best[q] == gq && gq > 0.0f) dsm_atom_min_u32(a_best + (uint32_t)((3 + q) * 32 + lane) * 4u, besth[q]);
    best[q] = gq;
  }
  sync_all();
  BPLX_STAMP(15);
#pragma unroll
  for (int q = 0; q < 3; q++) besth[q] = dsm_ld_u32(a_best + (uint32_t)((3 + q) * 32 + lane) * 4u);
  const bool noclip = CLIP && __all_sync(kFull, best[0] < 15.0f && best[1] < 15.0f) && !(kp.force_clip_forms & 2);
  const float Lam = fmaxf(best[0], best[1]);
  const int qlam = best[0] >= best[1] ? 0 : 1;
  bool s_need[2];
  uint32_t s_hoff[2], s_off0[2];
  uint4 s_hdr[2];
#pragma unroll
  for (int which = 0; which < 2; which++) {
    s_need[which] = (which == 0 || best[2] > 1.0f) && best[which == 0 ? qlam : 2] > 0.0f;
    s_hoff[which] = s_need[which] ? (which == 0 ? (qlam == 0 ? besth[0] : besth[1]) : besth[2]) : b1_0;
    const unsigned char* base = kp.stream1 + s_hoff[which];
    s_off0[which] = __ldg(reinterpret_cast<const uint32_t*>(base + 16 + (size_t)vwarp * ESZ));
    s_hdr[which] = __ldg(reinterpret_cast<const uint4*>(base));
  }
  const float LB = -1.0f / Lam;
  const float UB = fminf(1.0f / best[2], 1.0f);
  const float cc = fmaf(r, UB - LB, LB);

  BPLX_STAMP(4);
#pragma unroll
  for (int which = 0; which < 2; which++) {
    const bool need = s_need[which];
    const float target = which == 0 ? Lam : best[2];
    const int q = which == 0 ? qlam : 2;
    const unsigned char* ent = kp.stream1 + s_hoff[which] + 16;
    uint32_t off_next = s_off0[which];
    const Hdr L = unpack_hdr(s_hdr[which]);
    const uint32_t n = need ? L.n0 : 0u;
    float2 own = lds64(tab + (need ? L.own_off : 0u));
    if (L.kind >= kH0) { const float s = own.x; own.x = own.y; own.y = s; }
    const uint32_t nmax = __reduce_max_sync(kFull, n);
    uint32_t found = 0xffffffffu, info = 0u;
#pragma unroll 1
    for (uint32_t i = vwarp; i < nmax; i += VW) {
      const uint32_t off = off_next;
      if (i + VW < nmax) off_next = __ldg(reinterpret_cast<const uint32_t*>(ent + (size_t)(i + VW) * ESZ));
      if (i < n) {
        const float2 ea = lds64(tab + off);
        const float X = own.x * ea.x, Y = own.y * ea.y;
        float val;
        if (CLIP) {
          const float Xc = fminf(X, 15.0f), Yc = fminf(Y, 15.0f);
          val = q == 0 ? Xc : (q == 1 ? Yc : Xc * Yc);
        } else {
          val = q == 0 ? X : (q == 1 ? Y : (own.x * own.y) * (ea.x * ea.y));
        }
        if (val == target && found == 0xffffffffu) {
          found = (i << 24) | ((!CLIP || X < 15.0f) ? 1u << 23 : 0u) | ((!CLIP || Y < 15.0f) ? 1u << 22 : 0u) | off;
          info = L.vteam | (L.kind << 16);
        }
      }
    }
    if (found != 0xffffffffu) {
      dsm_atom_min_u32(a_found + (uint32_t)(which * 32 + lane) * 4u, found);
      dsm_st_u32(a_found + (uint32_t)(64 + which * 32 + lane) * 4u, info);
    }
  }

  BPLX_STAMP(5);
  float gc = 0.0f;
  {
    float g[6] = {0.0f, 0.0f, 0.0f, 0.0f, 0.0f, 0.0f}, cacc = 0.0f;
    const uint32_t nst = ring.num_stages();
    for (uint32_t k = 0; k < nst; k++) {
      uint32_t bytes;
      const uint32_t a0 = ring.acquire(k, &bytes);
      if (k == 0) BPLX_STAMP(18);
      uint32_t a = a0;
      const uint32_t aend = a0 + bytes;
      while (a + kp.min_piece2 <= aend) {
        const Hdr L = unpack_hdr(lds128u(a));
        a += 16;
        if (L.flags & kTeamFirst) {
#pragma unroll
          for (int e = 0; e < 6; e++) g[e] = 0.0f;
        }
        float2 own = lds64(tab + L.own_off);
        if (L.kind >= kH0) { const float s = own.x; own.x = own.y; own.y = s; }
        const bool home = (L.kind & 1) == 0;
        float lt, du, gx, gy;
        if (!CLIP) tau_piece<kTauPlain>(a, L, own, home, cc, tab, lt, du, gx, gy);
        else if (noclip) tau_piece<kTauUnclipped>(a, L, own, home, cc, tab, lt, du, gx, gy);
        else tau_piece<kTauClipped>(a, L, own, home, cc, tab, lt, du, gx, gy);
        if (home) {
          lp_acc = fmaf(lt, kLn2, lp_acc);
          gc += du;
        }
        add_own(g, L.kind, gx, gy);
        if (kp.Cf > 0) {
          cacc += L.kind == kH1 ? gx - gy : gy - gx;
          if (L.flags & kVteamLast) {
            if (ln.active) red_add(ln.sc + (size_t)L.vteam * kp.Cpad, cacc);
            cacc = 0.0f;
          }
        }
        if (L.flags & kTeamLast) {
          if (p2s) put_side(kp, p2_tab + (((L.kind & 1) * kp.T + L.team) * (2 + ndec)) * 32 + lane, g, hacc);
          else put_raw<true>(kp, ln, (int)L.team, g, hacc);
        }
      }
      ring.release(k);
    }
  }
  BPLX_STAMP(6);
  red_gc[warp * 32 + lane] = gc;
  __syncthreads();
  gc = 0.0f;
  for (int w = 0; w < W; w++) gc += red_gc[w * 32 + lane];
  if (S > 1) {
    if (warp == 0) dsm_st_f32(a_cl + (uint32_t)(crank * 32 + lane) * 4u, gc);
    cg::this_cluster().sync();
    gc = 0.0f;
    for (int q = 0; q < S; q++) gc += dsm_ld_f32(a_cl + (uint32_t)(q * 32 + lane) * 4u);
  }
  {
    const float t11 = fmaxf(1.0f - cc, 0.0f);
    gc -= kp.w11 / t11;
    if (vwarp == 0 && kp.w11 != 0.0f) lp_acc = fmaf(kp.w11, logf(t11), lp_acc);
  }

  BPLX_STAMP(7);
  Fixup fx;
  fx.h1 = 0u;
  fx.confs = 0u;
#pragma unroll
  for (int which = 0; which < 2; which++) {
    const uint32_t packed = dsm_ld_u32(a_found + (uint32_t)(which * 32 + lane) * 4u);
    fx.teams[which] = 0xffffffffu;
    fx.vts[which] = 0xffffffffu;
    fx.vx[which] = fx.vy[which] = 0.0f;
    if (packed != 0xffffffffu) {
      const uint32_t info = dsm_ld_u32(a_found + (uint32_t)(64 + which * 32 + lane) * 4u);
      const uint32_t f_off = packed & 0x3fffffu;
      const bool h1 = ((info >> 16) & 3u) == kH1;
      const uint32_t own_v = info & 0xffffu;
      const uint32_t opp_v = (f_off - (h1 ? kp.tabQ1 : kp.tabP0)) / kRowBytes;
      const bool xfree = (packed >> 23) & 1u, yfree = (packed >> 22) & 1u;
      if (which == 0) {
        const float wgt = gc * (1.0f - r) / Lam;
        fx.vx[0] = (qlam == 0 && xfree) ? wgt : 0.0f;
        fx.vy[0] = (qlam == 1 && yfree) ? wgt : 0.0f;
      } else {
        const float wgt = -gc * r / best[2];
        fx.vx[1] = xfree ? wgt : 0.0f;
        fx.vy[1] = yfree ? wgt : 0.0f;
      }
      fx.h1 |= (h1 ? 1u : 0u) << which;
      fx.vts[which] = own_v | (opp_v << 16);
      if (kp.Cf > 0)
        fx.confs |= ((uint32_t)__ldg(kp.v_conf + own_v) | ((uint32_t)__ldg(kp.v_conf + opp_v) << 8)) << (16 * which);
    }
  }

  BPLX_STAMP(8);
  const bool has_rho = !dc && !lik;
  const float pri = lik ? 0.0f : 1.0f;
  float u = 0.5f, rho = 0.0f, inv_s2 = 1.0f;
  if (has_rho) {
    u = red_hyp[11 * 32 + lane];
    rho = 2.0f * u - 1.0f;
    inv_s2 = 1.0f / (1.0f - rho * rho);
  }
  float a_mu_d = 0.0f, a_ls_a = 0.0f, a_ls_d = 0.0f, a_rho = 0.0f, a_mu[4], a_ls[4];
#pragma unroll
  for (int i = 0; i < 4; i++) a_mu[i] = a_ls[i] = 0.0f;
  {
    Hyp hy;
    hy.mu_d = red_hyp[0 * 32 + lane]; hy.sig_a = red_hyp[1 * 32 + lane]; hy.sig_d = red_hyp[2 * 32 + lane];
#pragma unroll
    for (int i = 0; i < 4; i++) { hy.mu[i] = red_hyp[(3 + i) * 32 + lane]; hy.sig[i] = red_hyp[(7 + i) * 32 + lane]; }

    for (int t = vwarp; t < kp.T; t += VW) {
      const float za = ln.ld(o.za + t), zd = ln.ld(o.zd + t);
      const uint32_t v0 = (uint32_t)__ldg(kp.team_vptr + t), nv = (uint32_t)__ldg(kp.team_vptr + t + 1) - v0;
      const float4 ys = __ldg(reinterpret_cast<const float4*>(kp.yteam + (size_t)t * 8));
      const float2 ys2 = __ldg(reinterpret_cast<const float2*>(kp.yteam + (size_t)t * 8 + 4));
      float ra = ld_cg(ln.g(o.za + t)) + ys.x;
      float rd = ld_cg(ln.g(o.zd + t)) + ys.y;
      float rx[4] = {ys.z, ys.w, ys2.x, ys2.y};
      float dec[4] = {0.0f, 0.0f, 0.0f, 0.0f};
#pragma unroll
      for (int i = 0; i < 4; i++) {
        if (i < ndec) {
          dec[i] = ln.ld(o.dec[i] + t);
          rx[i] += ld_cg(ln.g(o.dec[i] + t));
        }
      }
      if (p2s) {
#pragma unroll
        for (int side = 0; side < 2; side++) {
          const float* q = p2_tab + ((side * kp.T + t) * (2 + ndec)) * 32 + lane;
          ra += q[0];
          rd += q[32];
#pragma unroll
          for (int i = 0; i < 4; i++)
            if (i < ndec) rx[i] += q[(2 + i) * 32];
        }
      }
#pragma unroll
      for (int which = 0; which < 2; which++) {
        if ((fx.vts[which] & 0xffffu) - v0 < nv) fold_fixup(fx, which, 0, ra, rd, rx);
        if ((fx.vts[which] >> 16) - v0 < nv) fold_fixup(fx, which, 1, ra, rd, rx);
      }
      float p_za, p_zd;
      if (has_rho) {
        const float e = zd - rho * za;
        const float es = e * inv_s2;
        lp_acc -= 0.5f * (za * za + e * es);
        p_za = -za + rho * es;
        p_zd = -es;
        a_rho += es * za - rho * es * es + rho * inv_s2;
      } else {
        lp_acc -= pri * 0.5f * (za * za + zd * zd);
        p_za = -pri * za;
        p_zd = -pri * zd;
      }
      if (ln.active) {
        *ln.g(o.za + t) = fmaf(hy.sig_a, ra, p_za);
        *ln.g(o.zd + t) = fmaf(hy.sig_d, rd, p_zd);
      }
      a_ls_a = fmaf(hy.sig_a * za, ra, a_ls_a);
      a_ls_d = fmaf(hy.sig_d * zd, rd, a_ls_d);
      a_mu_d += rd;
      if (dc) a_mu[0] += rx[0];
#pragma unroll
      for (int i = 0; i < 4; i++) {
        if (i < ndec) {
          lp_acc -= pri * 0.5f * dec[i] * dec[i];
          if (ln.active) *ln.g(o.dec[i] + t) = fmaf(hy.sig[i], rx[i], -pri * dec[i]);
          a_mu[i] += rx[i];
          a_ls[i] = fmaf(hy.sig[i] * dec[i], rx[i], a_ls[i]);
        }
      }
      if (kp.K > 0) {
        dsm_st_f32(a_teamrows + (uint32_t)(t * 64 + lane) * 4u, ra);
        dsm_st_f32(a_teamrows + (uint32_t)(t * 64 + 32 + lane) * 4u, rd);
      }
    }
    if (dc) a_mu[0] += hacc;
  }
  for (int k = vwarp; k < kp.Cf; k += VW) {
    const float cf = ln.ld(o.conf + k);
    float s = __ldg(kp.yconf + k) - pri * cf;
    lp_acc -= pri * 0.5f * cf * cf;
    const int j0 = __ldg(kp.conf_vptr + k), j1 = __ldg(kp.conf_vptr + k + 1);
    for (int j = j0; j < j1; j++) s += ld_cg(ln.sc + (size_t)__ldg(kp.conf_vlist + j) * kp.Cpad);
#pragma unroll
    for (int ws = 0; ws < 4; ws++)
      if (fx.vts[ws >> 1] != 0xffffffffu && ((fx.confs >> (8 * ((ws >> 1) * 2 + (ws & 1)))) & 0xffu) == (uint32_t)k)
        s += fixup_conf(fx, ws >> 1, ws & 1);
    if (ln.active) *ln.g(o.conf + k) = s;
  }

  BPLX_STAMP(9);
  float* part = reinterpret_cast<float*>(smem + kp.epi_part);
  {
    float* p = part + (size_t)warp * kPartRows * 32 + lane;
    p[0 * 32] = lp_acc; p[1 * 32] = a_mu_d; p[2 * 32] = a_ls_a; p[3 * 32] = a_ls_d;
#pragma unroll
    for (int i = 0; i < 4; i++) { p[(4 + i) * 32] = a_mu[i]; p[(8 + i) * 32] = a_ls[i]; }
    p[12 * 32] = a_rho;
  }
  __syncthreads();
  if (S > 1) {
    for (int row = warp; row < kAccRows; row += W) {
      float s = 0.0f;
      for (int w = 0; w < W; w++) s += part[((size_t)w * kPartRows + row) * 32 + lane];
      dsm_st_f32(a_partcl + (uint32_t)((crank * kPartRows + row) * 32 + lane) * 4u, s);
    }
    cg::this_cluster().sync();
    if (crank != 0) return;
  }
  BPLX_STAMP(10);
  auto total = [&](int row) {
    float s = 0.0f;
    if (S > 1) {
      for (int q = 0; q < S; q++) s += dsm_ld_f32(a_partcl + (uint32_t)((q * kPartRows + row) * 32 + lane) * 4u);
    } else {
      for (int w = 0; w < W; w++) s += part[((size_t)w * kPartRows + row) * 32 + lane];
    }
    return s;
  };
  float lp = 0.0f;
  const int n_items = kp.nhyper + 2 + 2 * kp.K;
  for (int item = warp; item < n_items; item += W) {
    if (item < kp.nhyper) {
      const HyperDesc hd = kp.hyper[item];
      const float x = ln.ld(hd.off);
      const float acc = total(hd.row);
      float gval;
      if (hd.kind == 0) {
        const float z = (x - hd.loc) * hd.inv_scale;
        lp -= 0.5f * z * z;
        gval = fmaf(-z, hd.inv_scale, acc);
      } else if (hd.kind == 2) {
        gval = acc;
      } else {
        const float z = expf(x) * hd.inv_scale;
        lp += fmaf(-0.5f * z, z, x);
        gval = fmaf(-z, z, 1.0f) + acc;
      }
      if (ln.active) *ln.g(hd.off) = gval;
    } else if (item == kp.nhyper) {
      if (has_rho) {
        lp += 0.5f * (float)kp.T * logf(inv_s2) + 2.0f * logf(u) + 4.0f * logf(1.0f - u);
        if (ln.active) *ln.g(o.u) = 2.0f - 6.0f * u + total(12) * 2.0f * u * (1.0f - u);
      }
    } else if (item == kp.nhyper + 1) {
      lp += total(0) + (lik ? 0.0f : 2.0f * (logf(r) + logf(1.0f - r)));
      if (ln.active) {
        *ln.g(o.raw) = lik ? gc * (UB - LB) : 2.0f * (1.0f - 2.0f * r) + gc * r * (1.0f - r) * (UB - LB);
        if (kp.corr_coef) kp.corr_coef[chain] = cc;
      }
    } else {
      const int task = item - kp.nhyper - 2, k = task >> 1, isd = task & 1;
      const float* rows = reinterpret_cast<const float*>(smem + kp.epi_team) + isd * 32 + lane;
      const int d = (isd ? o.beta_d : o.beta_a) + k;
      const float b = ln.ld(d);
      float s = -b;
      lp -= 0.5f * b * b;
      for (int t = 0; t < kp.T; t++) s = fmaf(__ldg(kp.Xs + (size_t)t * kp.K + k), rows[(size_t)t * 64], s);
      if (ln.active) *ln.g(d) = s;
    }
  }
  BPLX_STAMP(11);
  red_gc[warp * 32 + lane] = lp;
  __syncthreads();
  if (warp == 0 && ln.active) {
    lp = kp.const_term;
    for (int w = 0; w < W; w++) lp += red_gc[w * 32 + lane];
    kp.lp[chain] = lp == INFINITY ? NAN : lp;
  }
}

template <bool CLIP>
static int launch_t(const KernelParams& kp, const WarpBounds& wb, cudaStream_t stream, bool set_attr, bool pdl) {
  auto* fn = &logdensity_kernel<CLIP>;
  if (set_attr) {
    BPLX_CUDA(cudaFuncSetAttribute(fn, cudaFuncAttributeMaxDynamicSharedMemorySize, 227 * 1024));
    return BPLX_OK;
  }
  cudaLaunchConfig_t cfg{};
  cfg.gridDim = dim3((unsigned)(kp.ngroups * kp.split));
  cfg.blockDim = dim3((unsigned)(kp.nwarps * 32));
  cfg.dynamicSmemBytes = kp.smem_total;
  cfg.stream = stream;
  cudaLaunchAttribute at[2];
  int na = 0;
  if (kp.split > 1) {
    at[na].id = cudaLaunchAttributeClusterDimension;
    at[na].val.clusterDim.x = (unsigned)kp.split;
    at[na].val.clusterDim.y = 1;
    at[na].val.clusterDim.z = 1;
    na++;
  }
  if (pdl && pdl_enabled()) {
    at[na].id = cudaLaunchAttributeProgrammaticStreamSerialization;
    at[na].val.programmaticStreamSerializationAllowed = 1;
    na++;
  }
  cfg.attrs = at;
  cfg.numAttrs = (unsigned)na;
  BPLX_CUDA(cudaLaunchKernelEx(&cfg, fn, kp, wb));
  BPLX_CUDA(cudaGetLastError());
  note_launch(1);
  return BPLX_OK;
}

template <bool CLIP>
static int max_clusters_t(const KernelParams& kp, int split) {
  cudaLaunchConfig_t cfg{};
  cfg.gridDim = dim3((unsigned)split);
  cfg.blockDim = dim3((unsigned)(kp.nwarps * 32));
  cfg.dynamicSmemBytes = kp.smem_total;
  cudaLaunchAttribute at[1];
  at[0].id = cudaLaunchAttributeClusterDimension;
  at[0].val.clusterDim.x = (unsigned)split;
  at[0].val.clusterDim.y = 1;
  at[0].val.clusterDim.z = 1;
  cfg.attrs = at;
  cfg.numAttrs = 1;
  int n = 0;
  if (cudaOccupancyMaxActiveClusters(&n, &logdensity_kernel<CLIP>, &cfg) != cudaSuccess) {
    cudaGetLastError();
    return 0;
  }
  return n;
}
int logdensity_max_clusters(const KernelParams& kp, int split) {
  return kp.clip ? max_clusters_t<true>(kp, split) : max_clusters_t<false>(kp, split);
}

#ifdef BPLX_TIMELINE
extern "C" int bplx_timeline_read(unsigned long long* out) {
  return cudaMemcpyFromSymbol(out, g_timeline, sizeof(g_timeline)) == cudaSuccess ? 0 : -1;
}
#endif

int logdensity_set_attributes(const KernelParams& kp) {
  static const WarpBounds none{};
  return kp.clip ? launch_t<true>(kp, none, nullptr, true, false) : launch_t<false>(kp, none, nullptr, true, false);
}
int launch_logdensity(const KernelParams& kp, const WarpBounds& wb, cudaStream_t stream, bool pdl) {
  return kp.clip ? launch_t<true>(kp, wb, stream, false, pdl) : launch_t<false>(kp, wb, stream, false, pdl);
}

}
```

bpl_next_b200/csrc/plan.cc:

```cpp
#include "plan.h"

#include <algorithm>
#include <cmath>
#include <cstdarg>
#include <cstdio>
#include <cstdlib>
#include <cstring>
#include <map>
#include <numeric>

namespace bplx {
namespace {

struct RawEntry {
  uint32_t opp;
  uint8_t cls;
  double w, wyx, wyy;
};

std::string fmt(const char* f, ...) {
  char buf[512];
  va_list ap;
  va_start(ap, f);
  vsnprintf(buf, sizeof buf, f, ap);
  va_end(ap);
  return buf;
}

void add_site(std::string* s, const char* name, int off, int count, const char* tr) {
  *s += fmt("%s:%d:%d:%s;", name, off, count, tr);
}

int make_layout(int model, int T, int K, int Cf, ThetaOffsets* o, std::string* s) {
  ThetaOffsets z;
  memset(&z, 0xff, sizeof z);
  int d = 0;
  auto scalar = [&](const char* n, const char* tr) { add_site(s, n, d, 1, tr); return d++; };
  auto vec = [&](const char* n, int cnt, const char* tr) {
    add_site(s, n, d, cnt, tr);
    int r = d;
    d += cnt;
    return r;
  };
  if (model == BPLX_DIXON_COLES) {
    z.mean[0] = scalar("home_advantage", "real");
    z.mean_defence = scalar("mean_defence", "real");
    z.log_std_attack = scalar("std_attack", "exp");
    z.log_std_defence = scalar("std_defence", "exp");
    z.za = vec("attack_decentered", T, "real");
    z.zd = vec("defence_decentered", T, "real");
    z.raw = scalar("corr_coef_raw", "sigmoid");
  } else if (model == BPLX_EXTENDED) {
    z.mean[0] = scalar("mean_home_advantage", "real");
    z.log_std[0] = scalar("std_home_advantage", "exp");
    z.mean_defence = scalar("mean_defence", "real");
    z.log_std_attack = scalar("std_attack", "exp");
    z.log_std_defence = scalar("std_defence", "exp");
    z.beta_a = vec("attack_coefficients", K, "real");
    z.beta_d = vec("defence_coefficients", K, "real");
    z.u = scalar("u", "sigmoid");
    z.za = vec("standardised_attack", T, "real");
    z.zd = vec("standardised_defence", T, "real");
    z.dec[0] = vec("home_advantage_decentered", T, "real");
    z.raw = scalar("corr_coef_raw", "sigmoid");
  } else if (model == BPLX_NEUTRAL || model == BPLX_NEUTRAL_WC) {
    static const char* nm[4] = {"home_attack", "away_attack", "home_defence", "away_defence"};
    z.mean_defence = scalar("mean_defence", "real");
    z.log_std_attack = scalar("std_attack", "exp");
    z.log_std_defence = scalar("std_defence", "exp");
    for (int i = 0; i < 4; i++) z.mean[i] = scalar((std::string("mean_") + nm[i]).c_str(), "real");
    for (int i = 0; i < 4; i++) z.log_std[i] = scalar((std::string("std_") + nm[i]).c_str(), "exp");
    z.u = scalar("u", "sigmoid");
    z.beta_a = vec("attack_coefficients", K, "real");
    z.beta_d = vec("defence_coefficients", K, "real");
    z.za = vec("standardised_attack", T, "real");
    z.zd = vec("standardised_defence", T, "real");
    for (int i = 0; i < 4; i++) z.dec[i] = vec((std::string(nm[i]) + "_decentered").c_str(), T, "real");
    if (model == BPLX_NEUTRAL_WC) z.conf = vec("confederation_strength_decentered", Cf, "real");
    z.raw = scalar("corr_coef_raw", "sigmoid");
  } else if (model == BPLX_DYNAMIC) {
    static const char* nm[4] = {"home_attack", "away_attack", "home_defence", "away_defence"};
    const int G = Cf;
    for (int i = 0; i < 4; i++) z.mean[i] = vec((std::string("mean_") + nm[i]).c_str(), G, "real");
    for (int i = 0; i < 4; i++) z.log_std[i] = vec((std::string("std_") + nm[i]).c_str(), G, "exp");
    z.log_std_attack = vec("std_attack", G, "exp");
    z.log_std_defence = vec("std_defence", G, "exp");
    z.mean_defence = scalar("mean_defence", "real");
    z.beta_a = vec("attack_coefficients", K, "real");
    z.beta_d = vec("defence_coefficients", K, "real");
    z.u = vec("u", G * T, "sigmoid");
    z.za = vec("standardised_attack", G * T, "real");
    z.zd = vec("standardised_defence", G * T, "real");
    for (int i = 0; i < 4; i++) z.dec[i] = vec((std::string(nm[i]) + "_decentered").c_str(), G * T, "real");
    z.raw = scalar("corr_coef_raw", "sigmoid");
  } else {
    return -1;
  }
  if (K == 0) z.beta_a = z.beta_d = -1;
  *o = z;
  return d;
}

}

static int build_plan_dynamic(const bplx_problem_desc& d, HostPlan* out, std::string* err, int force_warps);

int build_plan(const bplx_problem_desc& d, HostPlan* out, std::string* err, int force_warps) {
  const int model = d.model, M = d.num_matches, T = d.num_teams, K = d.num_covariates;
  const bool wc = model == BPLX_NEUTRAL_WC;
  const bool neutral = wc || model == BPLX_NEUTRAL;
  const int Cf = wc ? d.num_conferences : 0;
#define FAIL(code, ...)      \
  do {                       \
    *err = fmt(__VA_ARGS__); \
    return (code);           \
  } while (0)
  if (model < 0 || model > BPLX_DYNAMIC) FAIL(BPLX_E_INVALID, "unknown model %d", model);
  if (model == BPLX_DYNAMIC) return build_plan_dynamic(d, out, err, force_warps);
  if (M <= 0) FAIL(BPLX_E_INVALID, "num_matches must be positive (got %d)", M);
  if (T <= 0 || T > 65535) FAIL(BPLX_E_INVALID, "num_teams out of range (%d)", T);
  if (K < 0 || K > kMaxCov) FAIL(BPLX_E_UNSUPPORTED, "num_covariates %d outside [0, %d]", K, kMaxCov);
  if (K > 0 && model == BPLX_DIXON_COLES) FAIL(BPLX_E_INVALID, "DIXON_COLES takes no covariates");
  if (K > 0 && !d.covariates) FAIL(BPLX_E_INVALID, "covariates is NULL but num_covariates = %d", K);
  if (!d.home_team || !d.away_team || !d.home_goals || !d.away_goals)
    FAIL(BPLX_E_INVALID, "home_team / away_team / home_goals / away_goals must not be NULL");
  if (wc && (Cf <= 0 || Cf > 255 || !d.home_conf || !d.away_conf))
    FAIL(BPLX_E_INVALID, "NEUTRAL_WC needs home_conf, away_conf and 0 < num_conferences <= 255");
  for (int m = 0; m < M; m++) {
    if (d.home_team[m] >= T || d.away_team[m] >= T)
      FAIL(BPLX_E_INVALID, "team index out of range at match %d", m);
    if (wc && (d.home_conf[m] >= Cf || d.away_conf[m] >= Cf))
      FAIL(BPLX_E_INVALID, "confederation index out of range at match %d", m);
    if (d.weights && !(d.weights[m] >= 0.0f && d.weights[m] <= 3.0e38f))
      FAIL(BPLX_E_INVALID, "weights must be finite and non-negative (match %d)", m);
  }

  HostPlan& P = *out;
  KernelParams& kp = P.kp;
  kp.model = model;
  kp.T = T;
  kp.K = K;
  kp.Cf = Cf;
  kp.clip = model == BPLX_EXTENDED;
  kp.ndec = model == BPLX_DIXON_COLES ? 0 : (model == BPLX_EXTENDED ? 1 : 4);
  kp.D = make_layout(model, T, K, Cf, &kp.off, &P.layout);

  const double kLogSqrt2Pi = 0.91893853320467274178, kLog2 = 0.69314718055994530942;
  double const_term = 0.0;
  double const_lik = 0.0;
  {
    int n = 0;
    auto normal = [&](int off, int row, double loc, double scale) {
      kp.hyper[n++] = HyperDesc{off, row, 0, (float)loc, (float)(1.0 / scale)};
      const_term += -std::log(scale) - kLogSqrt2Pi;
    };
    auto halfnormal = [&](int off, int row, double scale) {
      kp.hyper[n++] = HyperDesc{off, row, 1, 0.0f, (float)(1.0 / scale)};
      const_term += -std::log(scale) - kLogSqrt2Pi + kLog2;
    };
    const double std_scale = neutral ? 0.5 : 1.0;
    normal(kp.off.mean_defence, 1, 0.0, 1.0);
    halfnormal(kp.off.log_std_attack, 2, std_scale);
    halfnormal(kp.off.log_std_defence, 3, std_scale);
    if (!neutral) {
      normal(kp.off.mean[0], 4, 0.1, 0.2);
      if (model == BPLX_EXTENDED) halfnormal(kp.off.log_std[0], 8, 1.0);
    } else {
      for (int i = 0; i < 4; i++) {
        normal(kp.off.mean[i], 4 + i, (i & 1) ? -0.1 : 0.1, 0.2);
        halfnormal(kp.off.log_std[i], 8 + i, 1.0);
      }
    }
    kp.nhyper = n;
    const_term -= (double)T * (2.0 + kp.ndec) * kLogSqrt2Pi;
    const_term -= (double)(Cf + 2 * K) * kLogSqrt2Pi;
    if (model != BPLX_DIXON_COLES) const_term += std::log(20.0);
    const_term += std::log(6.0);
  }

  std::map<std::pair<int, int>, int> vmap;
  if (wc) {
    for (int m = 0; m < M; m++) {
      vmap[{d.home_team[m], d.home_conf[m]}] = 0;
      vmap[{d.away_team[m], d.away_conf[m]}] = 0;
    }
  } else {
    for (int t = 0; t < T; t++) vmap[{t, 0}] = 0;
  }
  int V = 0;
  P.v_team.clear();
  P.v_conf.clear();
  for (auto& kv : vmap) {
    kv.second = V++;
    P.v_team.push_back((uint16_t)kv.first.first);
    P.v_conf.push_back((uint8_t)kv.first.second);
  }
  if (V > 65535) FAIL(BPLX_E_UNSUPPORTED, "too many (team, confederation) pairs (%d)", V);
  kp.V = V;
  P.team_vptr.assign(T + 1, 0);
  for (int v = 0; v < V; v++) P.team_vptr[P.v_team[v] + 1]++;
  for (int t = 0; t < T; t++) P.team_vptr[t + 1] += P.team_vptr[t];
  P.conf_vptr.assign(Cf + 1, 0);
  P.conf_vlist.assign(wc ? V : 0, 0);
  if (wc) {
    for (int v = 0; v < V; v++) P.conf_vptr[P.v_conf[v] + 1]++;
    for (int c = 0; c < Cf; c++) P.conf_vptr[c + 1] += P.conf_vptr[c];
    std::vector<int> fill(P.conf_vptr.begin(), P.conf_vptr.end() - 1);
    for (int v = 0; v < V; v++) P.conf_vlist[fill[P.v_conf[v]]++] = v;
  }

  bool has1 = false, has0 = false;
  for (int m = 0; m < M; m++) {
    bool nv = neutral && d.neutral_venue && d.neutral_venue[m];
    (nv ? has0 : has1) = true;
  }
  kp.has1 = has1;
  kp.has0 = has0;
  const uint32_t tab_rows = (uint32_t)V + 1;
  uint32_t off = 0;
  kp.tabP1 = kp.tabQ1 = kp.tabP0 = 0;
  if (has1) {
    kp.tabP1 = off;
    off += tab_rows * kRowBytes;
    kp.tabQ1 = off;
    off += tab_rows * kRowBytes;
  }
  if (has0) {
    kp.tabP0 = off;
    off += tab_rows * kRowBytes;
  }
  const uint32_t table_bytes = off;

  std::vector<std::vector<RawEntry>> raw1((size_t)V * 4), raw2((size_t)V * 4);
  std::vector<double> yexp((size_t)V * 6, 0.0);
  double w11 = 0.0;
  for (int m = 0; m < M; m++) {
    const int h = d.home_team[m], a = d.away_team[m];
    const int hc = wc ? d.home_conf[m] : 0, ac = wc ? d.away_conf[m] : 0;
    const int hv = vmap[{h, hc}], av = vmap[{a, ac}];
    const bool nv = neutral && d.neutral_venue && d.neutral_venue[m];
    const double w = d.weights ? (double)d.weights[m] : 1.0;
    const int yh = d.home_goals[m], ya = d.away_goals[m];
    const_term -= w * (std::lgamma(yh + 1.0) + std::lgamma(ya + 1.0));
    const_lik -= w * (std::lgamma(yh + 1.0) + std::lgamma(ya + 1.0));
    const int kh = nv ? kH0 : kH1, ka = nv ? kA0 : kA1;
    RawEntry eh{(uint32_t)av, 0, w, nv ? w * ya : w * yh, nv ? w * yh : w * ya};
    RawEntry ea{(uint32_t)hv, 0, w, w * yh, w * ya};
    raw1[(size_t)hv * 4 + kh].push_back(eh);
    raw1[(size_t)av * 4 + ka].push_back(ea);
    if (!kp.clip) {
      if (!nv) {
        yexp[(size_t)hv * 6 + eAh1] += w * yh;
        yexp[(size_t)hv * 6 + eBh1] += w * ya;
        yexp[(size_t)av * 6 + eBa1] += w * yh;
        yexp[(size_t)av * 6 + eAa1] += w * ya;
      } else {
        yexp[(size_t)hv * 6 + eA0] += w * yh;
        yexp[(size_t)hv * 6 + eB0] += w * ya;
        yexp[(size_t)av * 6 + eB0] += w * yh;
        yexp[(size_t)av * 6 + eA0] += w * ya;
      }
    }
    if (yh == 1 && ya == 1) {
      w11 += w;
    } else if (yh <= 1 && ya <= 1) {
      int cls_std = (yh == 0 && ya == 0) ? 0 : (yh == 1 ? 2  : 1 );
      int cls_h = cls_std;
      if (nv && cls_std != 0) cls_h = 3 - cls_std;
      eh.cls = (uint8_t)cls_h;
      ea.cls = (uint8_t)cls_std;
      raw2[(size_t)hv * 4 + kh].push_back(eh);
      raw2[(size_t)av * 4 + ka].push_back(ea);
    }
  }
  kp.w11 = (float)w11;
  kp.const_term = (float)const_term;
  {
    ThetaOffsets z;
    memset(&z, 0xff, sizeof z);
    int dd = 0;
    std::string& ls = P.lik_layout;
    auto vec = [&](const char* n, int cnt) {
      add_site(&ls, n, dd, cnt, "real");
      const int r0 = dd;
      dd += cnt;
      return r0;
    };
    z.za = vec("attack", T);
    z.zd = vec("defence", T);
    int nh = 0;
    if (model == BPLX_DIXON_COLES) {
      z.mean[0] = vec("home_advantage", 1);
      P.lik_hyper[nh++] = HyperDesc{z.mean[0], 4, 2, 0.0f, 1.0f};
    } else if (model == BPLX_EXTENDED) {
      z.dec[0] = vec("home_advantage", T);
    } else {
      static const char* nm[4] = {"home_attack", "away_attack", "home_defence", "away_defence"};
      for (int i = 0; i < 4; i++) z.dec[i] = vec(nm[i], T);
    }
    if (wc) z.conf = vec("confederation_strength", Cf);
    add_site(&ls, "corr_coef_raw", dd, 1, "unit");
    z.raw = dd++;
    P.lik_off = z;
    P.lik_nhyper = nh;
    P.lik_D = dd;
    P.lik_const = (float)const_lik;
  }
  P.yexp.resize(yexp.size());
  for (size_t i = 0; i < yexp.size(); i++) P.yexp[i] = (float)yexp[i];
  {
    std::vector<double> yt((size_t)T * 8, 0.0), yc((size_t)Cf, 0.0);
    for (int v = 0; v < V; v++) {
      const double* g = &yexp[(size_t)v * 6];
      double* o = &yt[(size_t)P.v_team[v] * 8];
      const double gA = g[eAh1] + g[eAa1] + g[eA0], gB = g[eBh1] + g[eBa1] + g[eB0];
      o[0] += gA;
      o[1] -= gB;
      o[2] += g[eAh1];
      o[3] += g[eAa1];
      o[4] -= g[eBh1];
      o[5] -= g[eBa1];
      if (wc) yc[P.v_conf[v]] += gA - gB;
    }
    P.yteam.resize(yt.size());
    for (size_t i = 0; i < yt.size(); i++) P.yteam[i] = (float)yt[i];
    P.yconf.resize(yc.size());
    for (size_t i = 0; i < yc.size(); i++) P.yconf[i] = (float)yc[i];
  }
  P.Xs.assign(d.covariates ? d.covariates : nullptr, d.covariates ? d.covariates + (size_t)T * K : nullptr);

  auto own_off = [&](int v, int kind) -> uint32_t {
    uint32_t base = kind == kH1 ? kp.tabP1 : kind == kA1 ? kp.tabQ1 : kp.tabP0;
    return base + (uint32_t)v * kRowBytes;
  };
  auto opp_base = [&](int kind) -> uint32_t { return kind == kH1 ? kp.tabQ1 : kind == kA1 ? kp.tabP1 : kp.tabP0; };

  auto merge = [](std::vector<RawEntry>& v) {
    std::stable_sort(v.begin(), v.end(), [](const RawEntry& a, const RawEntry& b) {
      return a.cls != b.cls ? a.cls < b.cls : a.opp < b.opp;
    });
    size_t o = 0;
    for (size_t i = 0; i < v.size(); i++) {
      if (o && v[o - 1].cls == v[i].cls && v[o - 1].opp == v[i].opp) {
        v[o - 1].w += v[i].w;
        v[o - 1].wyx += v[i].wyx;
        v[o - 1].wyy += v[i].wyy;
      } else {
        v[o++] = v[i];
      }
    }
    v.resize(o);
  };
  for (auto& v : raw1) merge(v);
  for (auto& v : raw2) merge(v);
  P.team_flags.assign(T, 0);
  for (int v = 0; v < V; v++)
    for (int k = 0; k < 4; k++)
      if (!raw1[(size_t)v * 4 + k].empty()) P.team_flags[P.v_team[v]] |= 1;

  auto team_costs = [&](const std::vector<std::vector<RawEntry>>& raw, double per_entry, double per_list,
                        double per_team) {
    std::vector<double> cost(T, 0.0);
    for (int v = 0; v < V; v++)
      for (int k = 0; k < 4; k++) {
        const size_t n = raw[(size_t)v * 4 + k].size();
        if (n) cost[P.v_team[v]] += per_list * (1.0 + (double)n / 100.0) + per_entry * (double)n;
      }
    for (int t = 0; t < T; t++)
      if (cost[t] > 0.0) cost[t] += per_team;
    return cost;
  };
  auto assign = [&](const std::vector<double>& cost, int W, std::vector<std::vector<int>>* teams) {
    std::vector<int> order(T);
    std::iota(order.begin(), order.end(), 0);
    std::stable_sort(order.begin(), order.end(), [&](int a, int b) { return cost[a] > cost[b]; });
    std::vector<double> load(W, 0.0);
    teams->assign(W, {});
    for (int t : order) {
      if (cost[t] == 0.0) continue;
      int best = 0;
      for (int w = 1; w < W; w++)
        if (load[w] < load[best]) best = w;
      load[best] += cost[t];
      (*teams)[best].push_back(t);
    }
    for (auto& v : *teams) std::sort(v.begin(), v.end());
    return *std::max_element(load.begin(), load.end());
  };
  const std::vector<double> cost1 = team_costs(raw1, kp.clip ? 16.0 : 6.0, 40.0, 30.0);
  const std::vector<double> cost2 = team_costs(raw2, 12.0, 60.0, 30.0);
  auto smem_need = [&](int W, uint32_t stage) {
    const uint32_t epi = (K > 0 ? (uint32_t)T * kRowBytes : 0u) + (uint32_t)(W + kMaxSplit) * kPartRows * 128u;
    const uint32_t tabb = (std::max(table_bytes, epi) + 127u) / 128u * 128u;
    return tabb + (uint32_t)W * kStages * stage + 128u + (uint32_t)W * kStages * 8u + 3u * 256u + 2u * 128u + 2u * 128u +
           12u * 128u + (uint32_t)(W + kMaxSplit) * 128u;
  };
  const uint32_t kSmemMax = 227u * 1024u;
  int W = 0;
  uint32_t stage = 1024;
  std::vector<std::vector<int>> w1, w2;
  if (force_warps <= 0) {
    if (const char* e = getenv("BPLX_NWARPS")) force_warps = atoi(e);
  }
  if (const char* e = getenv("BPLX_STAGE")) stage = (uint32_t)atoi(e) == 512u ? 512u : 1024u;
  if (force_warps > 0) {
    W = std::max(1, std::min(force_warps, kMaxWarps));
    if (smem_need(W, stage) > kSmemMax) stage = 512;
  } else {
    double best = 0.0;
    for (int cand : {4, 8, 12, 16, 20, 24}) {
      if (cand > kMaxWarps) continue;
      uint32_t st = stage;
      if (smem_need(cand, st) > kSmemMax) st = 512;
      if (smem_need(cand, st) > kSmemMax) continue;
      std::vector<std::vector<int>> t1, t2;
      const double span = assign(cost1, cand, &t1) + assign(cost2, cand, &t2) + 4.0 * cand + (st == 512 ? 0.05 * best : 0.0);
      if (W == 0 || span < 0.97 * best) best = span, W = cand, stage = st;
    }
    if (W == 0) W = 4, stage = 512;
  }
  kp.nwarps = W;
  kp.stage_bytes = stage;
  kp.force_clip_forms = 0;
  if (const char* e = getenv("BPLX_CLIP_FORMS")) kp.force_clip_forms = atoi(e);
  {
    std::vector<std::vector<int>> t1, t2;
    const double span = assign(cost1, W, &t1) + assign(cost2, W, &t2);
    kp.split_hint = span >= 32000.0 ? 8 : span >= 16000.0 ? 4 : span >= 8000.0 ? 2 : 1;
  }

  std::vector<std::vector<int>> w2_items;
  kp.smem_p2 = 0;
  {
    std::vector<std::pair<int, double>> units;
    for (int t = 0; t < T; t++)
      for (int side = 0; side < 2; side++) {
        double c = 0.0;
        for (int v = P.team_vptr[t]; v < P.team_vptr[t + 1]; v++)
          for (int k = side; k < 4; k += 2) {
            const size_t n = raw2[(size_t)v * 4 + k].size();
            if (n) c += 60.0 * (1.0 + (double)n / 100.0) + 12.0 * (double)n;
          }
        if (c > 0.0) units.push_back({t * 4 + (1 << side), c + 30.0});
      }
    std::stable_sort(units.begin(), units.end(), [](const auto& a, const auto& b) { return a.second > b.second; });
    std::vector<double> load(W, 0.0);
    std::vector<std::vector<int>> items(W);
    for (const auto& u : units) {
      int best = 0;
      for (int w = 1; w < W; w++)
        if (load[w] < load[best]) best = w;
      load[best] += u.second;
      items[best].push_back(u.first);
    }
    for (auto& v : items) std::sort(v.begin(), v.end());
    std::vector<std::vector<int>> t2;
    const double span_team = assign(cost2, W, &t2);
    const double span_unit = units.empty() ? 0.0 : *std::max_element(load.begin(), load.end());
    const uint32_t p2_bytes = 2u * (uint32_t)T * (uint32_t)(2 + kp.ndec) * 128u;
    const bool off = getenv("BPLX_NO_P2SPLIT") != nullptr;
    if (!off && Cf <= 0 && span_unit < 0.85 * span_team && smem_need(W, stage) + p2_bytes <= kSmemMax) {
      w2_items = items;
      kp.smem_p2 = 1;
    }
  }

  const uint32_t zero_row = (uint32_t)V * kRowBytes;
  auto put = [](std::vector<unsigned char>* s, const void* p, size_t n) {
    const unsigned char* b = static_cast<const unsigned char*>(p);
    s->insert(s->end(), b, b + n);
  };
  auto emit = [&](int Wtot, std::vector<unsigned char>* s1, std::vector<unsigned char>* s2, std::vector<uint32_t>* wb1,
                  std::vector<uint32_t>* wb2) {
  const bool by_side = kp.smem_p2 != 0 && Wtot == kp.nwarps;
  const int W = Wtot;
  assign(cost1, W, &w1);
  assign(cost2, W, &w2);
  std::vector<std::vector<int>> it1(W), it2(W);
  for (int w = 0; w < W; w++) {
    for (int t : w1[w]) it1[w].push_back(t * 4 + 3);
    for (int t : w2[w]) it2[w].push_back(t * 4 + 3);
  }
  if (by_side) it2 = w2_items;
  P.n1 = P.n2 = P.n1_padded = P.n2_padded = P.nlists1 = P.nlists2 = 0;
  wb1->assign(W + 1, 0);
  wb2->assign(W + 1, 0);
  for (int phase = 1; phase <= 2; phase++) {
    const auto& raw = phase == 1 ? raw1 : raw2;
    const auto& by_warp = phase == 1 ? it1 : it2;
    std::vector<unsigned char>& S = phase == 1 ? *s1 : *s2;
    std::vector<uint32_t>& wb = phase == 1 ? *wb1 : *wb2;
    const size_t esz = (phase == 1 && kp.clip) ? sizeof(EntryClip) : sizeof(Entry);
    const size_t gran = 16;
    const size_t min_piece = sizeof(ListHdr) + gran;
    (phase == 1 ? kp.min_piece1 : kp.min_piece2) = (uint32_t)min_piece;
    S.clear();
    for (int w = 0; w < W; w++) {
      const size_t wstart = S.size();
      for (int item : by_warp[w]) {
        const int t = item >> 2, sides = item & 3;
        size_t team_first_hdr = (size_t)-1, last_hdr = 0;
        for (int v = P.team_vptr[t]; v < P.team_vptr[t + 1]; v++) {
          size_t vteam_last_hdr = (size_t)-1;
          for (int k = 0; k < 4; k++) {
            const auto& r = raw[(size_t)v * 4 + k];
            if (r.empty() || !((sides >> (k & 1)) & 1)) continue;
            (phase == 1 ? P.n1 : P.n2) += (long long)r.size();
            std::vector<unsigned char> body;
            std::vector<uint8_t> cls;
            if (phase == 1) {
              for (const RawEntry& e : r) {
                const uint32_t o = opp_base(k) + e.opp * kRowBytes;
                if (kp.clip) {
                  EntryClip x{o, (float)e.w, (float)e.wyx, (float)e.wyy};
                  put(&body, &x, sizeof x);
                } else {
                  Entry x{o, (float)e.w};
                  put(&body, &x, sizeof x);
                }
                cls.push_back(0);
              }
              while (!kp.clip && (cls.size() & 1)) {
                Entry x{opp_base(k) + zero_row, 0.0f};
                put(&body, &x, sizeof x);
                cls.push_back(0);
              }
            } else {
              size_t i = 0;
              for (int c = 0; c < 3; c++) {
                const uint32_t comp = c == 2 ? 4u : 0u;
                size_t cnt = 0;
                for (; i < r.size() && r[i].cls == c; i++, cnt++) {
                  Entry x{opp_base(k) + r[i].opp * kRowBytes + comp, (float)r[i].w};
                  put(&body, &x, sizeof x);
                  cls.push_back((uint8_t)c);
                }
                if (cnt & 1) {
                  Entry x{opp_base(k) + zero_row + comp, 0.0f};
                  put(&body, &x, sizeof x);
                  cls.push_back((uint8_t)c);
                }
              }
            }
            (phase == 1 ? P.n1_padded : P.n2_padded) += (long long)cls.size();
            size_t done = 0;
            while (done < cls.size()) {
              size_t in_stage = (S.size() - wstart) % stage;
              if (stage - in_stage < min_piece) {
                S.resize(S.size() + (stage - in_stage), 0);
                in_stage = 0;
              }
              const size_t space = stage - in_stage - sizeof(ListHdr);
              const size_t take = std::min(cls.size() - done, space / gran * gran / esz);
              ListHdr H{};
              H.own_off = own_off(v, k);
              H.vteam = (uint16_t)v;
              H.kind = (uint8_t)k;
              H.team = (uint16_t)t;
              uint16_t cnt[3] = {0, 0, 0};
              for (size_t i = done; i < done + take; i++) cnt[cls[i]]++;
              H.n0 = cnt[0];
              H.n1 = cnt[1];
              H.n2 = cnt[2];
              const size_t hdr_at = S.size();
              put(&S, &H, sizeof H);
              put(&S, body.data() + done * esz, take * esz);
              done += take;
              (phase == 1 ? P.nlists1 : P.nlists2)++;
              if (team_first_hdr == (size_t)-1) team_first_hdr = hdr_at;
              vteam_last_hdr = last_hdr = hdr_at;
            }
          }
          if (vteam_last_hdr != (size_t)-1) reinterpret_cast<ListHdr*>(&S[vteam_last_hdr])->flags |= kVteamLast;
        }
        if (team_first_hdr != (size_t)-1) {
          reinterpret_cast<ListHdr*>(&S[team_first_hdr])->flags |= kTeamFirst;
          reinterpret_cast<ListHdr*>(&S[last_hdr])->flags |= kTeamLast;
        }
      }
      wb[w + 1] = (uint32_t)S.size();
    }
    if (S.empty()) S.resize(16, 0);
  }
  };
  for (int i = kNumSplits - 1; i >= 1; i--)
    emit(W << i, &P.more[i - 1].stream1, &P.more[i - 1].stream2, &P.more[i - 1].warp_b1, &P.more[i - 1].warp_b2);
  emit(W, &P.stream1, &P.stream2, &P.warp_b1, &P.warp_b2);

  kp.epi_team = 0;
  kp.epi_part = K > 0 ? (uint32_t)T * kRowBytes : 0u;
  kp.epi_cl = kp.epi_part + (uint32_t)W * kPartRows * 128u;
  const uint32_t epi = kp.epi_cl + (uint32_t)kMaxSplit * kPartRows * 128u;
  kp.tab_bytes = (std::max(table_bytes, epi) + 127u) / 128u * 128u;
  kp.smem_ring = kp.tab_bytes;
  kp.smem_bar = kp.smem_ring + (uint32_t)W * kStages * stage;
  kp.smem_red = (kp.smem_bar + (uint32_t)W * kStages * 8u + 127u) / 128u * 128u;
  kp.smem_red_cl = kp.smem_red + 3u * 256u + 2u * 128u + 2u * 128u + 12u * 128u + (uint32_t)W * 128u;
  kp.smem_total = kp.smem_red_cl + (uint32_t)kMaxSplit * 128u;
  if (kp.smem_p2) {
    kp.smem_p2 = kp.smem_total;
    kp.smem_total += 2u * (uint32_t)T * (uint32_t)(2 + kp.ndec) * 128u;
  }
  if (kp.smem_total > kSmemMax)
    FAIL(BPLX_E_UNSUPPORTED, "problem needs %u bytes of shared memory per CTA (max %u): too many (team, confederation) pairs (%d)",
         kp.smem_total, kSmemMax, V);
#undef FAIL
  return BPLX_OK;
}

#include "plan_dynamic.inc"

}
```

bpl_next_b200/csrc/plan.h:

```cpp
#pragma once
#include <stdint.h>

#include <string>
#include <vector>

#include "../../include/bplx.h"

namespace bplx {

constexpr int kChains = 32;
constexpr int kRowBytes = 256;
constexpr int kMaxCov = 16;
constexpr int kMaxWarps = 24;
constexpr int kMaxWarpsDyn = 20;
constexpr int kStages = 2;
constexpr int kAccRows = 13;
constexpr int kPartRows = 16;
constexpr int kMaxSplit = 8;
constexpr int kNumSplits = 4;

enum Kind : uint8_t { kH1 = 0, kA1 = 1, kH0 = 2, kA0 = 3 };
enum Exponent : int { eAh1 = 0, eBh1 = 1, eBa1 = 2, eAa1 = 3, eA0 = 4, eB0 = 5 };

constexpr uint8_t kTeamFirst = 1;
constexpr uint8_t kTeamLast = 2;
constexpr uint8_t kVteamLast = 4;
constexpr uint8_t kGwFirst = 8;
constexpr uint8_t kStageEnd = 16;
constexpr uint8_t kPhase2 = 32;

struct Entry {
  uint32_t off;
  float w;
};
struct EntryClip {
  uint32_t off;
  float w;
  float wyx;
  float wyy;
};

struct ListHdr {
  uint32_t own_off;
  uint16_t vteam;
  uint8_t kind;
  uint8_t flags;
  uint16_t n0;
  uint16_t n1;
  uint16_t n2;
  uint16_t team;
};
static_assert(sizeof(ListHdr) == 16, "ListHdr must be 16 bytes");

struct ThetaOffsets {
  int mean_defence, log_std_attack, log_std_defence;
  int mean[4];
  int log_std[4];
  int u;
  int beta_a, beta_d;
  int za, zd;
  int dec[4];
  int conf;
  int raw;
};

struct HyperDesc {
  int off;
  int row;
  int kind;
  float loc, inv_scale;
};

struct WarpBounds {
  uint32_t b1[kMaxSplit * kMaxWarps + 1], b2[kMaxSplit * kMaxWarps + 1];
};

struct KernelParams {
  int model, T, K, Cf, V;
  int G;
  int as_written;
  int D, nwarps;
  int ndec;
  int clip;
  int lik_only;
  int has1, has0;
  uint32_t tabP1, tabQ1, tabP0;
  uint32_t tab_bytes;
  uint32_t stage_bytes;
  uint32_t min_piece1, min_piece2;
  uint32_t smem_ring, smem_bar, smem_red, smem_total;
  uint32_t epi_team, epi_part;
  uint32_t epi_cl;
  uint32_t smem_red_cl;
  uint32_t smem_p2;
  uint32_t dyn_state, dyn_part, dyn_hyp, dyn_fin;
  int dyn_nbuf;
  int dyn_hyp_ws;
  int split_hint;
  int group0, ngroups;
  int force_clip_forms;
  ThetaOffsets off;
  const unsigned char* stream1;
  const unsigned char* stream2;
  const uint32_t* warp_b1;
  const uint32_t* warp_b2;
  const int32_t* team_vptr;
  const uint8_t* team_flags;
  const uint16_t* v_team;
  const uint8_t* v_conf;
  const int32_t* conf_vptr;
  const int32_t* conf_vlist;
  const float* yexp;
  const float* yteam;
  const float* yconf;
  const float* Xs;
  const int32_t* gw_tptr;
  const uint16_t* gw_tlist;
  HyperDesc hyper[12];
  int nhyper;
  float w11;
  float const_term;
  int C;
  int split;
  int sd, sc;
  const float* theta;
  float* lp;
  float* grad;
  float* corr_coef;
  float* scratch;
  int Cpad;
};

struct SplitStreams {
  std::vector<unsigned char> stream1, stream2;
  std::vector<uint32_t> warp_b1, warp_b2;
};

struct HostPlan {
  KernelParams kp{};
  ThetaOffsets lik_off{};
  HyperDesc lik_hyper[12]{};
  int lik_nhyper = 0, lik_D = 0;
  float lik_const = 0.0f;
  std::string lik_layout;
  std::vector<unsigned char> stream1, stream2;
  std::vector<uint32_t> warp_b1, warp_b2;
  SplitStreams more[kNumSplits - 1];
  std::vector<int32_t> team_vptr, conf_vptr, conf_vlist;
  std::vector<uint8_t> team_flags;
  std::vector<uint16_t> v_team;
  std::vector<uint8_t> v_conf;
  std::vector<float> yexp, yteam, yconf, Xs;
  std::vector<int32_t> gw_tptr;
  std::vector<uint16_t> gw_tlist;
  std::string layout;
  long long n1 = 0, n2 = 0, n1_padded = 0, n2_padded = 0, nlists1 = 0, nlists2 = 0;
};

int build_plan(const bplx_problem_desc& d, HostPlan* out, std::string* err, int force_warps = 0);

}
```

Baseline: 816.8 billion.

## Move away-side rate lists into phase two and rebalance warp work

Phase one now processes only the home-side rate lists, which need the max-tracking for clipping. The away-side rate lists are placed after a new per-warp boundary and handled in the second phase, interleaved with the tau lists. Odd and even warps take the two segments in opposite order, and the host planner assigns teams using per-phase cost estimates. The aim is to shorten phase one and balance load across the sync point, at the cost of more complex stream layout and accumulation paths (put_side now adds instead of storing).

Result: faster. 839.1 billion, median of 6 (+2.7%).

```diff
diff --git a/bpl_next_b200/csrc/api.cu b/bpl_next_b200/csrc/api.cu
--- a/bpl_next_b200/csrc/api.cu
+++ b/bpl_next_b200/csrc/api.cu
@@ -262,13 +262,15 @@
     UP(more[i - 1].warp_b1, p->wb1[i]);
     UP(more[i - 1].warp_b2, p->wb2[i]);
   }
-  auto keep_bounds = [&](int i, const std::vector<uint32_t>& b1, const std::vector<uint32_t>& b2) {
+  auto keep_bounds = [&](int i, const std::vector<uint32_t>& b1, const std::vector<uint32_t>& bh,
+                         const std::vector<uint32_t>& b2) {
     const size_t cap = sizeof(p->wb[i].b1) / sizeof(uint32_t);
     for (size_t k = 0; k < b1.size() && k < cap; k++) p->wb[i].b1[k] = b1[k];
+    for (size_t k = 0; k < bh.size() && k + 1 < cap; k++) p->wb[i].bh[k] = bh[k];
     for (size_t k = 0; k < b2.size() && k < cap; k++) p->wb[i].b2[k] = b2[k];
   };
-  keep_bounds(0, hp.warp_b1, hp.warp_b2);
-  for (int i = 1; i < kNumSplits; i++) keep_bounds(i, hp.more[i - 1].warp_b1, hp.more[i - 1].warp_b2);
+  keep_bounds(0, hp.warp_b1, hp.warp_bh, hp.warp_b2);
+  for (int i = 1; i < kNumSplits; i++) keep_bounds(i, hp.more[i - 1].warp_b1, hp.more[i - 1].warp_bh, hp.more[i - 1].warp_b2);
   kp.stream1 = p->s1[0];
   kp.stream2 = p->s2[0];
   kp.warp_b1 = p->wb1[0];
@@ -303,15 +305,22 @@
   p->stats[7] = kp.V;
   if (kp.model != BPLX_DYNAMIC) {
     p->warp_stats.assign((size_t)kp.nwarps * 12, 0);
-    for (int phase = 0; phase < 2; phase++) {
-      const std::vector<unsigned char>& S = phase ? hp.stream2 : hp.stream1;
-      const std::vector<uint32_t>& wb = phase ? hp.warp_b2 : hp.warp_b1;
-      const size_t esz = (phase == 0 && kp.clip) ? sizeof(EntryClip) : sizeof(Entry);
-      const uint32_t minp = phase ? kp.min_piece2 : kp.min_piece1;
+    for (int st_i = 0; st_i < 2; st_i++) {
+      const std::vector<unsigned char>& S = st_i ? hp.stream2 : hp.stream1;
+      const std::vector<uint32_t>& wb = st_i ? hp.warp_b2 : hp.warp_b1;
+      const uint32_t minp = st_i ? kp.min_piece2 : kp.min_piece1;
       for (int w = 0; w < kp.nwarps && w + 1 < (int)wb.size(); w++) {
-        long long* o = &p->warp_stats[(size_t)w * 12 + phase * 6];
+        long long* o1 = &p->warp_stats[(size_t)w * 12];
+        long long* o2 = o1 + 4;
         const uint32_t len = wb[w + 1] - wb[w];
-        o[5] = (len + kp.stage_bytes - 1) / kp.stage_bytes;
+        const uint32_t nst = (len + kp.stage_bytes - 1) / kp.stage_bytes;
+        if (st_i) {
+          o2[7] += nst;
+        } else {
+          const uint32_t home_st = (hp.warp_bh[w] - wb[w] + kp.stage_bytes - 1) / kp.stage_bytes;
+          o1[3] = home_st;
+          o2[7] += nst - (hp.warp_bh[w] - wb[w]) / kp.stage_bytes;
+        }
         for (uint32_t st = 0; st < len; st += kp.stage_bytes) {
           uint32_t a = wb[w] + st;
           const uint32_t aend = wb[w] + std::min(len, st + kp.stage_bytes);
@@ -319,17 +328,20 @@
             ListHdr H;
             memcpy(&H, &S[a], sizeof H);
             if (H.n0 + H.n1 + H.n2 == 0) break;
-            const bool home = (H.kind & 1) == 0;
-            if (phase == 0) {
-              o[home ? 0 : 1]++;
-              o[home ? 2 : 3] += H.n0;
+            size_t esz = sizeof(Entry);
+            if (st_i) {
+              o2[0]++;
+              o2[1] += H.n0;
+              o2[2] += H.n1;
+              o2[3] += H.n2;
+              if (H.flags & kTeamFirst) o2[6]++;
             } else {
-              o[0]++;
-              o[1] += H.n0;
-              o[2] += H.n1;
-              o[3] += H.n2;
+              esz = kp.clip ? sizeof(EntryClip) : sizeof(Entry);
+              const bool home = (H.kind & 1) == 0;
+              (home ? o1[0] : o2[4])++;
+              (home ? o1[1] : o2[5]) += H.n0;
+              if (H.flags & kTeamFirst) o1[2]++;
             }
-            if (H.flags & kTeamFirst) o[4]++;
             a += (uint32_t)sizeof(ListHdr) + (uint32_t)((H.n0 + H.n1 + H.n2) * esz);
           }
         }
diff --git a/bpl_next_b200/csrc/k1_common.cuh b/bpl_next_b200/csrc/k1_common.cuh
--- a/bpl_next_b200/csrc/k1_common.cuh
+++ b/bpl_next_b200/csrc/k1_common.cuh
@@ -128,13 +128,13 @@
 }
 
 __device__ __forceinline__ void put_side(const KernelParams& kp, float* q, const float (&g)[6], float& hacc) {
-  q[0] = g[eAh1] + g[eAa1] + g[eA0];
-  q[32] = -(g[eBh1] + g[eBa1] + g[eB0]);
+  q[0] += g[eAh1] + g[eAa1] + g[eA0];
+  q[32] += -(g[eBh1] + g[eBa1] + g[eB0]);
   const float rx[4] = {g[eAh1], g[eAa1], -g[eBh1], -g[eBa1]};
   if (kp.ndec == 0) hacc += rx[0];
 #pragma unroll
   for (int i = 0; i < 4; i++)
-    if (i < kp.ndec) q[(2 + i) * 32] = rx[i];
+    if (i < kp.ndec) q[(2 + i) * 32] += rx[i];
 }
 
 struct Ring {
diff --git a/bpl_next_b200/csrc/logdensity.cu b/bpl_next_b200/csrc/logdensity.cu
--- a/bpl_next_b200/csrc/logdensity.cu
+++ b/bpl_next_b200/csrc/logdensity.cu
@@ -107,8 +107,8 @@
   Ring ring;
   ring.init(smem_u32(smem) + kp.smem_ring + warp * (kStages * kp.stage_bytes),
             smem_u32(smem) + kp.smem_bar + warp * (kStages * 8), kp.stage_bytes, lane);
-  const uint32_t b1_0 = wb.b1[vwarp], b1_1 = wb.b1[vwarp + 1];
-  ring.begin(kp.stream1 + b1_0, b1_1 - b1_0);
+  const uint32_t b1_0 = wb.b1[vwarp], bh = wb.bh[vwarp];
+  ring.begin(kp.stream1 + b1_0, bh - b1_0);
   pdl_wait();
   pdl_launch_dependents();
   ln.th = after_wait(ln.th);
@@ -223,6 +223,7 @@
           if (i < ndec) *ln.g(o.dec[i] + t) = 0.0f;
       }
       for (int v = in.v0; v < in.v1; v++) {
+        if (kp.Cf > 0 && (in.fl & 2) && ln.active && crank == 0) ln.sc[(size_t)v * kp.Cpad] = 0.0f;
         const float cf = kp.Cf > 0 ? ln.ld(o.conf + __ldg(kp.v_conf + v)) : 0.0f;
         float ex[6];
         ex[eAh1] = att + x[0] + cf;
@@ -282,52 +283,35 @@
         }
         float2 own = lds64(tab + L.own_off);
         if (L.kind >= kH0) { const float s = own.x; own.x = own.y; own.y = s; }
-        const bool home = (L.kind & 1) == 0;
         float gx, gy;
         if (!CLIP) {
           float2 acc0 = make_float2(0.0f, 0.0f), acc1 = acc0;
-          if (home) {
-            float m1 = 0.0f, m2 = 0.0f, m3 = 0.0f;
-            walk16(a, e_end, [&](const uint32_t at) {
-              const uint4 q = lds128u(at);
-              const float2 ea = lds64(tab + q.x), eb = lds64(tab + q.z);
-              acc0 = fma2(bc2(__uint_as_float(q.y)), ea, acc0);
-              acc1 = fma2(bc2(__uint_as_float(q.w)), eb, acc1);
-              m1 = fmaxf(m1, fmaxf(ea.x, eb.x));
-              m2 = fmaxf(m2, fmaxf(ea.y, eb.y));
-              m3 = fmaxf(m3, fmaxf(ea.x * ea.y, eb.x * eb.y));
-            });
-            const float v0 = own.x * m1, v1 = own.y * m2, v2 = (own.x * own.y) * m3;
-            if (v0 > best[0]) { best[0] = v0; besth[0] = hoff; }
-            if (v1 > best[1]) { best[1] = v1; besth[1] = hoff; }
-            if (v2 > best[2]) { best[2] = v2; besth[2] = hoff; }
-          } else {
-            walk16(a, e_end, [&](const uint32_t at) {
-              const uint4 q = lds128u(at);
-              const float2 ea = lds64(tab + q.x), eb = lds64(tab + q.z);
-              acc0 = fma2(bc2(__uint_as_float(q.y)), ea, acc0);
-              acc1 = fma2(bc2(__uint_as_float(q.w)), eb, acc1);
-            });
-          }
+          float m1 = 0.0f, m2 = 0.0f, m3 = 0.0f;
+          walk16(a, e_end, [&](const uint32_t at) {
+            const uint4 q = lds128u(at);
+            const float2 ea = lds64(tab + q.x), eb = lds64(tab + q.z);
+            acc0 = fma2(bc2(__uint_as_float(q.y)), ea, acc0);
+            acc1 = fma2(bc2(__uint_as_float(q.w)), eb, acc1);
+            m1 = fmaxf(m1, fmaxf(ea.x, eb.x));
+            m2 = fmaxf(m2, fmaxf(ea.y, eb.y));
+            m3 = fmaxf(m3, fmaxf(ea.x * ea.y, eb.x * eb.y));
+          });
+          const float v0 = own.x * m1, v1 = own.y * m2, v2 = (own.x * own.y) * m3;
+          if (v0 > best[0]) { best[0] = v0; besth[0] = hoff; }
+          if (v1 > best[1]) { best[1] = v1; besth[1] = hoff; }
+          if (v2 > best[2]) { best[2] = v2; besth[2] = hoff; }
           const float SX = own.x * (acc0.x + acc1.x), SY = own.y * (acc0.y + acc1.y);
           lp_acc -= 0.5f * (SX + SY);
           gx = -SX;
           gy = -SY;
         } else {
           float lp = 0.0f, m1 = 0.0f, m2 = 0.0f, m3 = 0.0f;
-          if (fast1) {
-            if (home) rate_piece_clip<true, true>(a, e_end, own, tab, lp, m1, m2, m3, gx, gy);
-            else rate_piece_clip<true, false>(a, e_end, own, tab, lp, m1, m2, m3, gx, gy);
-          } else {
-            if (home) rate_piece_clip<false, true>(a, e_end, own, tab, lp, m1, m2, m3, gx, gy);
-            else rate_piece_clip<false, false>(a, e_end, own, tab, lp, m1, m2, m3, gx, gy);
-          }
-          if (home) {
-            lp_acc += lp;
-            if (m1 > best[0]) { best[0] = m1; besth[0] = hoff; }
-            if (m2 > best[1]) { best[1] = m2; besth[1] = hoff; }
-            if (m3 > best[2]) { best[2] = m3; besth[2] = hoff; }
-          }
+          if (fast1) rate_piece_clip<true, true>(a, e_end, own, tab, lp, m1, m2, m3, gx, gy);
+          else rate_piece_clip<false, true>(a, e_end, own, tab, lp, m1, m2, m3, gx, gy);
+          lp_acc += lp;
+          if (m1 > best[0]) { best[0] = m1; besth[0] = hoff; }
+          if (m2 > best[1]) { best[1] = m2; besth[1] = hoff; }
+          if (m3 > best[2]) { best[2] = m3; besth[2] = hoff; }
         }
         add_own(g, L.kind, gx, gy);
         if (kp.Cf > 0) {
@@ -343,8 +327,18 @@
       ring.release(k);
     }
   }
-  const uint32_t b2_0 = wb.b2[vwarp], b2_1 = wb.b2[vwarp + 1];
-  ring.begin(kp.stream2 + b2_0, b2_1 - b2_0);
+  const bool rates_first = (vwarp & 1) == 0;
+  auto begin_segment = [&](const bool rates) -> uint32_t {
+    if (!rates) {
+      const uint32_t b2_0 = wb.b2[vwarp], b2_1 = wb.b2[vwarp + 1];
+      ring.begin(kp.stream2 + b2_0, b2_1 - b2_0);
+      return 0u;
+    }
+    const uint32_t s0 = bh - (bh - b1_0) % ring.S, b1_1 = wb.b1[vwarp + 1];
+    ring.begin(kp.stream1 + s0, b1_1 - s0);
+    return bh - s0;
+  };
+  uint32_t skip = begin_segment(rates_first);
 
   BPLX_STAMP(3);
 #pragma unroll
@@ -424,45 +418,69 @@
   float gc = 0.0f;
   {
     float g[6] = {0.0f, 0.0f, 0.0f, 0.0f, 0.0f, 0.0f}, cacc = 0.0f;
-    const uint32_t nst = ring.num_stages();
-    for (uint32_t k = 0; k < nst; k++) {
-      uint32_t bytes;
-      const uint32_t a0 = ring.acquire(k, &bytes);
-      if (k == 0) BPLX_STAMP(18);
-      uint32_t a = a0;
-      const uint32_t aend = a0 + bytes;
-      while (a + kp.min_piece2 <= aend) {
-        const Hdr L = unpack_hdr(lds128u(a));
-        a += 16;
-        if (L.flags & kTeamFirst) {
-#pragma unroll
-          for (int e = 0; e < 6; e++) g[e] = 0.0f;
-        }
-        float2 own = lds64(tab + L.own_off);
-        if (L.kind >= kH0) { const float s = own.x; own.x = own.y; own.y = s; }
-        const bool home = (L.kind & 1) == 0;
-        float lt, du, gx, gy;
-        if (!CLIP) tau_piece<kTauPlain>(a, L, own, home, cc, tab, lt, du, gx, gy);
-        else if (noclip) tau_piece<kTauUnclipped>(a, L, own, home, cc, tab, lt, du, gx, gy);
-        else tau_piece<kTauClipped>(a, L, own, home, cc, tab, lt, du, gx, gy);
-        if (home) {
-          lp_acc = fmaf(lt, kLn2, lp_acc);
-          gc += du;
-        }
-        add_own(g, L.kind, gx, gy);
-        if (kp.Cf > 0) {
-          cacc += L.kind == kH1 ? gx - gy : gy - gx;
-          if (L.flags & kVteamLast) {
-            if (ln.active) red_add(ln.sc + (size_t)L.vteam * kp.Cpad, cacc);
-            cacc = 0.0f;
+    for (int seg = 0; seg < 2; seg++) {
+      const bool rates = (seg == 0) == rates_first;
+      if (seg == 1) skip = begin_segment(rates);
+      const uint32_t nst = ring.num_stages();
+      for (uint32_t k = 0; k < nst; k++) {
+        uint32_t bytes;
+        const uint32_t a0 = ring.acquire(k, &bytes);
+        if (k == 0 && seg == 0) BPLX_STAMP(18);
+        uint32_t a = a0 + (k == 0 ? skip : 0u);
+        const uint32_t aend = a0 + bytes;
+        while (a + kp.min_piece2 <= aend) {
+          const Hdr L = unpack_hdr(lds128u(a));
+          a += 16;
+          float2 own = lds64(tab + L.own_off);
+          if (L.kind >= kH0) { const float s = own.x; own.x = own.y; own.y = s; }
+          float gx, gy;
+          if (!rates) {
+            const bool home = (L.kind & 1) == 0;
+            float lt, du;
+            if (!CLIP) tau_piece<kTauPlain>(a, L, own, home, cc, tab, lt, du, gx, gy);
+            else if (noclip) tau_piece<kTauUnclipped>(a, L, own, home, cc, tab, lt, du, gx, gy);
+            else tau_piece<kTauClipped>(a, L, own, home, cc, tab, lt, du, gx, gy);
+            if (home) {
+              lp_acc = fmaf(lt, kLn2, lp_acc);
+              gc += du;
+            }
+          } else {
+            const uint32_t e_end = a + L.n0 * ESZ;
+            if (!CLIP) {
+              float2 acc0 = make_float2(0.0f, 0.0f), acc1 = acc0;
+              walk16(a, e_end, [&](const uint32_t at) {
+                const uint4 q = lds128u(at);
+                const float2 ea = lds64(tab + q.x), eb = lds64(tab + q.z);
+                acc0 = fma2(bc2(__uint_as_float(q.y)), ea, acc0);
+                acc1 = fma2(bc2(__uint_as_float(q.w)), eb, acc1);
+              });
+              const float SX = own.x * (acc0.x + acc1.x), SY = own.y * (acc0.y + acc1.y);
+              lp_acc -= 0.5f * (SX + SY);
+              gx = -SX;
+              gy = -SY;
+            } else {
+              float lp, m1, m2, m3;
+              if (noclip) rate_piece_clip<true, false>(a, e_end, own, tab, lp, m1, m2, m3, gx, gy);
+              else rate_piece_clip<false, false>(a, e_end, own, tab, lp, m1, m2, m3, gx, gy);
+            }
           }
-        }
-        if (L.flags & kTeamLast) {
-          if (p2s) put_side(kp, p2_tab + (((L.kind & 1) * kp.T + L.team) * (2 + ndec)) * 32 + lane, g, hacc);
-          else put_raw<true>(kp, ln, (int)L.team, g, hacc);
-        }
-      }
-      ring.release(k);
+          add_own(g, L.kind, gx, gy);
+          if (kp.Cf > 0) {
+            cacc += L.kind == kH1 ? gx - gy : gy - gx;
+            if (L.flags & kVteamLast) {
+              if (ln.active) red_add(ln.sc + (size_t)L.vteam * kp.Cpad, cacc);
+              cacc = 0.0f;
+            }
+          }
+          if (L.flags & (rates ? kVteamLast : kTeamLast)) {
+            if (p2s) put_side(kp, p2_tab + (((L.kind & 1) * kp.T + L.team) * (2 + ndec)) * 32 + lane, g, hacc);
+            else put_raw<true>(kp, ln, (int)L.team, g, hacc);
+#pragma unroll
+            for (int e = 0; e < 6; e++) g[e] = 0.0f;
+          }
+        }
+        ring.release(k);
+      }
     }
   }
   BPLX_STAMP(6);
@@ -673,7 +691,7 @@
       lp += total(0) + (lik ? 0.0f : 2.0f * (logf(r) + logf(1.0f - r)));
       if (ln.active) {
         *ln.g(o.raw) = lik ? gc * (UB - LB) : 2.0f * (1.0f - 2.0f * r) + gc * r * (1.0f - r) * (UB - LB);
-        if (kp.corr_coef) kp.corr_coef[chain] = cc;
+        if (kp.corr_coef) kp.corr_coef[chain_raw] = cc;
       }
     } else {
       const int task = item - kp.nhyper - 2, k = task >> 1, isd = task & 1;
@@ -692,7 +710,7 @@
   if (warp == 0 && ln.active) {
     lp = kp.const_term;
     for (int w = 0; w < W; w++) lp += red_gc[w * 32 + lane];
-    kp.lp[chain] = lp == INFINITY ? NAN : lp;
+    kp.lp[chain_raw] = lp == INFINITY ? NAN : lp;
   }
 }
 
diff --git a/bpl_next_b200/csrc/plan.cc b/bpl_next_b200/csrc/plan.cc
--- a/bpl_next_b200/csrc/plan.cc
+++ b/bpl_next_b200/csrc/plan.cc
@@ -353,21 +353,29 @@
   };
   for (auto& v : raw1) merge(v);
   for (auto& v : raw2) merge(v);
+  auto in_phase1 = [](int k) { return (k & 1) == 0; };
   P.team_flags.assign(T, 0);
-  for (int v = 0; v < V; v++)
-    for (int k = 0; k < 4; k++)
-      if (!raw1[(size_t)v * 4 + k].empty()) P.team_flags[P.v_team[v]] |= 1;
-
-  auto team_costs = [&](const std::vector<std::vector<RawEntry>>& raw, double per_entry, double per_list,
-                        double per_team) {
+  for (int v = 0; v < V; v++) {
+    const bool p1 = !raw1[(size_t)v * 4 + kH1].empty() || !raw1[(size_t)v * 4 + kH0].empty();
+    P.team_flags[P.v_team[v]] |= p1 ? 1 : 2;
+  }
+
+  const double kHomeEntry = kp.clip ? 18.0 : 6.0, kAwayEntry = kp.clip ? 14.0 : 4.5, kTauEntry = 12.0;
+  const double kRateList = 40.0, kTauList = 60.0, kPerTeam = 30.0;
+  auto list_cost = [&](int v, int k, int phase) {
+    double c = 0.0;
+    const size_t n1 = raw1[(size_t)v * 4 + k].size(), n2 = raw2[(size_t)v * 4 + k].size();
+    if (n1 && in_phase1(k) == (phase == 1))
+      c += kRateList * (1.0 + (double)n1 / 100.0) + (in_phase1(k) ? kHomeEntry : kAwayEntry) * (double)n1;
+    if (n2 && phase == 2) c += kTauList * (1.0 + (double)n2 / 100.0) + kTauEntry * (double)n2;
+    return c;
+  };
+  auto team_costs = [&](int phase) {
     std::vector<double> cost(T, 0.0);
     for (int v = 0; v < V; v++)
-      for (int k = 0; k < 4; k++) {
-        const size_t n = raw[(size_t)v * 4 + k].size();
-        if (n) cost[P.v_team[v]] += per_list * (1.0 + (double)n / 100.0) + per_entry * (double)n;
-      }
+      for (int k = 0; k < 4; k++) cost[P.v_team[v]] += list_cost(v, k, phase);
     for (int t = 0; t < T; t++)
-      if (cost[t] > 0.0) cost[t] += per_team;
+      if (cost[t] > 0.0) cost[t] += kPerTeam;
     return cost;
   };
   auto assign = [&](const std::vector<double>& cost, int W, std::vector<std::vector<int>>* teams) {
@@ -387,8 +395,7 @@
     for (auto& v : *teams) std::sort(v.begin(), v.end());
     return *std::max_element(load.begin(), load.end());
   };
-  const std::vector<double> cost1 = team_costs(raw1, kp.clip ? 16.0 : 6.0, 40.0, 30.0);
-  const std::vector<double> cost2 = team_costs(raw2, 12.0, 60.0, 30.0);
+  const std::vector<double> cost1 = team_costs(1), cost2 = team_costs(2);
   auto smem_need = [&](int W, uint32_t stage) {
     const uint32_t epi = (K > 0 ? (uint32_t)T * kRowBytes : 0u) + (uint32_t)(W + kMaxSplit) * kPartRows * 128u;
     const uint32_t tabb = (std::max(table_bytes, epi) + 127u) / 128u * 128u;
@@ -437,11 +444,8 @@
       for (int side = 0; side < 2; side++) {
         double c = 0.0;
         for (int v = P.team_vptr[t]; v < P.team_vptr[t + 1]; v++)
-          for (int k = side; k < 4; k += 2) {
-            const size_t n = raw2[(size_t)v * 4 + k].size();
-            if (n) c += 60.0 * (1.0 + (double)n / 100.0) + 12.0 * (double)n;
-          }
-        if (c > 0.0) units.push_back({t * 4 + (1 << side), c + 30.0});
+          for (int k = side; k < 4; k += 2) c += list_cost(v, k, 2);
+        if (c > 0.0) units.push_back({t * 4 + (1 << side), c + kPerTeam});
       }
     std::stable_sort(units.begin(), units.end(), [](const auto& a, const auto& b) { return a.second > b.second; });
     std::vector<double> load(W, 0.0);
@@ -471,7 +475,7 @@
     s->insert(s->end(), b, b + n);
   };
   auto emit = [&](int Wtot, std::vector<unsigned char>* s1, std::vector<unsigned char>* s2, std::vector<uint32_t>* wb1,
-                  std::vector<uint32_t>* wb2) {
+                  std::vector<uint32_t>* wbh, std::vector<uint32_t>* wb2) {
   const bool by_side = kp.smem_p2 != 0 && Wtot == kp.nwarps;
   const int W = Wtot;
   assign(cost1, W, &w1);
@@ -484,108 +488,116 @@
   if (by_side) it2 = w2_items;
   P.n1 = P.n2 = P.n1_padded = P.n2_padded = P.nlists1 = P.nlists2 = 0;
   wb1->assign(W + 1, 0);
+  wbh->assign(W, 0);
   wb2->assign(W + 1, 0);
-  for (int phase = 1; phase <= 2; phase++) {
-    const auto& raw = phase == 1 ? raw1 : raw2;
-    const auto& by_warp = phase == 1 ? it1 : it2;
-    std::vector<unsigned char>& S = phase == 1 ? *s1 : *s2;
-    std::vector<uint32_t>& wb = phase == 1 ? *wb1 : *wb2;
-    const size_t esz = (phase == 1 && kp.clip) ? sizeof(EntryClip) : sizeof(Entry);
-    const size_t gran = 16;
-    const size_t min_piece = sizeof(ListHdr) + gran;
-    (phase == 1 ? kp.min_piece1 : kp.min_piece2) = (uint32_t)min_piece;
-    S.clear();
-    for (int w = 0; w < W; w++) {
-      const size_t wstart = S.size();
-      for (int item : by_warp[w]) {
-        const int t = item >> 2, sides = item & 3;
-        size_t team_first_hdr = (size_t)-1, last_hdr = 0;
-        for (int v = P.team_vptr[t]; v < P.team_vptr[t + 1]; v++) {
-          size_t vteam_last_hdr = (size_t)-1;
-          for (int k = 0; k < 4; k++) {
-            const auto& r = raw[(size_t)v * 4 + k];
-            if (r.empty() || !((sides >> (k & 1)) & 1)) continue;
-            (phase == 1 ? P.n1 : P.n2) += (long long)r.size();
-            std::vector<unsigned char> body;
-            std::vector<uint8_t> cls;
-            if (phase == 1) {
-              for (const RawEntry& e : r) {
-                const uint32_t o = opp_base(k) + e.opp * kRowBytes;
-                if (kp.clip) {
-                  EntryClip x{o, (float)e.w, (float)e.wyx, (float)e.wyy};
-                  put(&body, &x, sizeof x);
-                } else {
-                  Entry x{o, (float)e.w};
-                  put(&body, &x, sizeof x);
-                }
-                cls.push_back(0);
-              }
-              while (!kp.clip && (cls.size() & 1)) {
-                Entry x{opp_base(k) + zero_row, 0.0f};
-                put(&body, &x, sizeof x);
-                cls.push_back(0);
-              }
+  const size_t gran = 16;
+  const size_t min_piece = sizeof(ListHdr) + gran;
+  kp.min_piece1 = kp.min_piece2 = (uint32_t)min_piece;
+  s1->clear();
+  s2->clear();
+  enum Part { kHomeRates, kAwayRates, kTau };
+  auto put_item = [&](std::vector<unsigned char>& S, size_t wstart, int item, Part part) {
+    const int t = item >> 2, sides = item & 3;
+    const bool tau = part == kTau;
+    const size_t esz = (!tau && kp.clip) ? sizeof(EntryClip) : sizeof(Entry);
+    size_t team_first_hdr = (size_t)-1, last_hdr = 0;
+    for (int v = P.team_vptr[t]; v < P.team_vptr[t + 1]; v++) {
+      size_t vteam_last_hdr = (size_t)-1;
+      for (int k = 0; k < 4; k++) {
+        if (!((sides >> (k & 1)) & 1) || (part == kHomeRates && !in_phase1(k)) || (part == kAwayRates && in_phase1(k)))
+          continue;
+        const auto& r = (tau ? raw2 : raw1)[(size_t)v * 4 + k];
+        if (r.empty()) continue;
+        (tau ? P.n2 : P.n1) += (long long)r.size();
+        std::vector<unsigned char> body;
+        std::vector<uint8_t> cls;
+        if (!tau) {
+          for (const RawEntry& e : r) {
+            const uint32_t o = opp_base(k) + e.opp * kRowBytes;
+            if (kp.clip) {
+              EntryClip x{o, (float)e.w, (float)e.wyx, (float)e.wyy};
+              put(&body, &x, sizeof x);
             } else {
-              size_t i = 0;
-              for (int c = 0; c < 3; c++) {
-                const uint32_t comp = c == 2 ? 4u : 0u;
-                size_t cnt = 0;
-                for (; i < r.size() && r[i].cls == c; i++, cnt++) {
-                  Entry x{opp_base(k) + r[i].opp * kRowBytes + comp, (float)r[i].w};
-                  put(&body, &x, sizeof x);
-                  cls.push_back((uint8_t)c);
-                }
-                if (cnt & 1) {
-                  Entry x{opp_base(k) + zero_row + comp, 0.0f};
-                  put(&body, &x, sizeof x);
-                  cls.push_back((uint8_t)c);
-                }
-              }
+              Entry x{o, (float)e.w};
+              put(&body, &x, sizeof x);
             }
-            (phase == 1 ? P.n1_padded : P.n2_padded) += (long long)cls.size();
-            size_t done = 0;
-            while (done < cls.size()) {
-              size_t in_stage = (S.size() - wstart) % stage;
-              if (stage - in_stage < min_piece) {
-                S.resize(S.size() + (stage - in_stage), 0);
-                in_stage = 0;
-              }
-              const size_t space = stage - in_stage - sizeof(ListHdr);
-              const size_t take = std::min(cls.size() - done, space / gran * gran / esz);
-              ListHdr H{};
-              H.own_off = own_off(v, k);
-              H.vteam = (uint16_t)v;
-              H.kind = (uint8_t)k;
-              H.team = (uint16_t)t;
-              uint16_t cnt[3] = {0, 0, 0};
-              for (size_t i = done; i < done + take; i++) cnt[cls[i]]++;
-              H.n0 = cnt[0];
-              H.n1 = cnt[1];
-              H.n2 = cnt[2];
-              const size_t hdr_at = S.size();
-              put(&S, &H, sizeof H);
-              put(&S, body.data() + done * esz, take * esz);
-              done += take;
-              (phase == 1 ? P.nlists1 : P.nlists2)++;
-              if (team_first_hdr == (size_t)-1) team_first_hdr = hdr_at;
-              vteam_last_hdr = last_hdr = hdr_at;
+            cls.push_back(0);
+          }
+          while (!kp.clip && (cls.size() & 1)) {
+            Entry x{opp_base(k) + zero_row, 0.0f};
+            put(&body, &x, sizeof x);
+            cls.push_back(0);
+          }
+        } else {
+          size_t i = 0;
+          for (int c = 0; c < 3; c++) {
+            const uint32_t comp = c == 2 ? 4u : 0u;
+            size_t cnt = 0;
+            for (; i < r.size() && r[i].cls == c; i++, cnt++) {
+              Entry x{opp_base(k) + r[i].opp * kRowBytes + comp, (float)r[i].w};
+              put(&body, &x, sizeof x);
+              cls.push_back((uint8_t)c);
+            }
+            if (cnt & 1) {
+              Entry x{opp_base(k) + zero_row + comp, 0.0f};
+              put(&body, &x, sizeof x);
+              cls.push_back((uint8_t)c);
             }
           }
-          if (vteam_last_hdr != (size_t)-1) reinterpret_cast<ListHdr*>(&S[vteam_last_hdr])->flags |= kVteamLast;
         }
-        if (team_first_hdr != (size_t)-1) {
-          reinterpret_cast<ListHdr*>(&S[team_first_hdr])->flags |= kTeamFirst;
-          reinterpret_cast<ListHdr*>(&S[last_hdr])->flags |= kTeamLast;
+        (tau ? P.n2_padded : P.n1_padded) += (long long)cls.size();
+        size_t done = 0;
+        while (done < cls.size()) {
+          size_t in_stage = (S.size() - wstart) % stage;
+          if (stage - in_stage < min_piece) {
+            S.resize(S.size() + (stage - in_stage), 0);
+            in_stage = 0;
+          }
+          const size_t space = stage - in_stage - sizeof(ListHdr);
+          const size_t take = std::min(cls.size() - done, space / gran * gran / esz);
+          ListHdr H{};
+          H.own_off = own_off(v, k);
+          H.vteam = (uint16_t)v;
+          H.kind = (uint8_t)k;
+          H.team = (uint16_t)t;
+          uint16_t cnt[3] = {0, 0, 0};
+          for (size_t i = done; i < done + take; i++) cnt[cls[i]]++;
+          H.n0 = cnt[0];
+          H.n1 = cnt[1];
+          H.n2 = cnt[2];
+          const size_t hdr_at = S.size();
+          put(&S, &H, sizeof H);
+          put(&S, body.data() + done * esz, take * esz);
+          done += take;
+          (tau ? P.nlists2 : P.nlists1)++;
+          if (team_first_hdr == (size_t)-1) team_first_hdr = hdr_at;
+          vteam_last_hdr = last_hdr = hdr_at;
         }
       }
-      wb[w + 1] = (uint32_t)S.size();
-    }
-    if (S.empty()) S.resize(16, 0);
-  }
+      if (vteam_last_hdr != (size_t)-1) reinterpret_cast<ListHdr*>(&S[vteam_last_hdr])->flags |= kVteamLast;
+    }
+    if (team_first_hdr != (size_t)-1 && part != kAwayRates) {
+      reinterpret_cast<ListHdr*>(&S[team_first_hdr])->flags |= kTeamFirst;
+      reinterpret_cast<ListHdr*>(&S[last_hdr])->flags |= kTeamLast;
+    }
+  };
+  for (int w = 0; w < W; w++) {
+    size_t wstart = s1->size();
+    for (int item : it1[w]) put_item(*s1, wstart, item, kHomeRates);
+    (*wbh)[w] = (uint32_t)s1->size();
+    for (int item : it2[w]) put_item(*s1, wstart, item, kAwayRates);
+    (*wb1)[w + 1] = (uint32_t)s1->size();
+    wstart = s2->size();
+    for (int item : it2[w]) put_item(*s2, wstart, item, kTau);
+    (*wb2)[w + 1] = (uint32_t)s2->size();
+  }
+  if (s1->empty()) s1->resize(16, 0);
+  if (s2->empty()) s2->resize(16, 0);
   };
   for (int i = kNumSplits - 1; i >= 1; i--)
-    emit(W << i, &P.more[i - 1].stream1, &P.more[i - 1].stream2, &P.more[i - 1].warp_b1, &P.more[i - 1].warp_b2);
-  emit(W, &P.stream1, &P.stream2, &P.warp_b1, &P.warp_b2);
+    emit(W << i, &P.more[i - 1].stream1, &P.more[i - 1].stream2, &P.more[i - 1].warp_b1, &P.more[i - 1].warp_bh,
+         &P.more[i - 1].warp_b2);
+  emit(W, &P.stream1, &P.stream2, &P.warp_b1, &P.warp_bh, &P.warp_b2);
 
   kp.epi_team = 0;
   kp.epi_part = K > 0 ? (uint32_t)T * kRowBytes : 0u;
diff --git a/bpl_next_b200/csrc/plan.h b/bpl_next_b200/csrc/plan.h
--- a/bpl_next_b200/csrc/plan.h
+++ b/bpl_next_b200/csrc/plan.h
@@ -73,6 +73,7 @@
 
 struct WarpBounds {
   uint32_t b1[kMaxSplit * kMaxWarps + 1], b2[kMaxSplit * kMaxWarps + 1];
+  uint32_t bh[kMaxSplit * kMaxWarps];
 };
 
 struct KernelParams {
@@ -133,7 +134,7 @@
 
 struct SplitStreams {
   std::vector<unsigned char> stream1, stream2;
-  std::vector<uint32_t> warp_b1, warp_b2;
+  std::vector<uint32_t> warp_b1, warp_bh, warp_b2;
 };
 
 struct HostPlan {
@@ -144,7 +145,7 @@
   float lik_const = 0.0f;
   std::string lik_layout;
   std::vector<unsigned char> stream1, stream2;
-  std::vector<uint32_t> warp_b1, warp_b2;
+  std::vector<uint32_t> warp_b1, warp_bh, warp_b2;
   SplitStreams more[kNumSplits - 1];
   std::vector<int32_t> team_vptr, conf_vptr, conf_vlist;
   std::vector<uint8_t> team_flags;
```
